# seqan/slimm

Hardware: AMD Instinct MI355X
Metric: M alignment-records/sec -> final profile (higher is better)
Workload: dtype u32

## Files before the change

slimm_amd/csrc/kernels.h:

```cpp
#pragma once
#include <hip/hip_runtime.h>
#include <stdint.h>

#include <string>
#include <vector>

#include "record_filter.h"
#include "tile_plan.h"

#if defined(__HIP_DEVICE_COMPILE__)
#define SLIMM_PIN_VGPR(x) asm volatile("" : "+v"(x))
#else
#define SLIMM_PIN_VGPR(x) (void)(x)
#endif

namespace slimm {

enum {
    CNT_V = 0,
    CNT_M = 1,
    CNT_P = 2,
    CNT_ERR = 3,
    CNT_PAIRS = 4,
    CNT_REDO = 5,
    CNT_ITEMS = 10,
    CNT_ITEMS2 = 6,
    CNT_ANYGB = 8,
    CNT_MODE = 7,
    CNT_SPLIT = 9,
    CNT_FALLBACK = 11,
    CNT_PEAK = 13,
    CNT_WORDS = 32
};
enum { ERR_REF_RANGE = 1, ERR_RUN_LENGTH = 2, ERR_PAIR_OVERFLOW = 4, ERR_KEY_COLLISION = 8 };

#if defined(__HIPCC__)
__device__ __forceinline__ uint32_t wave_sum_dpp(uint32_t v) {
    v += __builtin_amdgcn_update_dpp(0u, v, 0x111, 0xf, 0xf, true);
    v += __builtin_amdgcn_update_dpp(0u, v, 0x112, 0xf, 0xf, true);
    v += __builtin_amdgcn_update_dpp(0u, v, 0x114, 0xf, 0xf, true);
    v += __builtin_amdgcn_update_dpp(0u, v, 0x118, 0xf, 0xf, true);
    v += __builtin_amdgcn_update_dpp(0u, v, 0x142, 0xa, 0xf, true);
    v += __builtin_amdgcn_update_dpp(0u, v, 0x143, 0xc, 0xf, true);
    return __builtin_amdgcn_readlane(v, 63);
}
#endif

struct PackArgs {
    const uint32_t* src[4] = {nullptr, nullptr, nullptr, nullptr};
    uint32_t n[4] = {0, 0, 0, 0};
    uint32_t reps[4] = {1, 1, 1, 1};
    int sum_k = -1;
    const uint32_t* sum_off = nullptr;
    const uint32_t* sum_idx = nullptr;
};
constexpr uint32_t kPackBytes8 = 0xffffffffu;
#ifdef __HIPCC__
__device__ __forceinline__ uint32_t packed_word(const PackArgs& pack, int k, uint32_t i) {
    uint32_t v = 0;
    if (k == pack.sum_k) {
        for (uint32_t j = pack.sum_off[i]; j < pack.sum_off[i + 1]; ++j) v += pack.src[k][pack.sum_idx[j]];
    } else if (pack.reps[k] == kPackBytes8) {
        const uint2 b = reinterpret_cast<const uint2*>(pack.src[k])[i];
#pragma unroll
        for (int l = 0; l < 4; ++l) {
            v |= ((b.x >> (8 * l)) & 0xffu) ? (1u << l) : 0u;
            v |= ((b.y >> (8 * l)) & 0xffu) ? (16u << l) : 0u;
        }
    } else {
        for (uint32_t rep = 0; rep < pack.reps[k]; ++rep) v |= pack.src[k][static_cast<size_t>(rep) * pack.n[k] + i];
    }
    return v;
}
#endif
constexpr uint32_t kMarkBytes = 8;
struct ZeroArgs {
    uint32_t* p[5] = {nullptr, nullptr, nullptr, nullptr, nullptr};
    uint32_t n[5] = {0, 0, 0, 0, 0};
    uint64_t* p64 = nullptr;
    uint32_t n64 = 0;
    uint32_t* cp_dst = nullptr;
    const uint32_t* cp_src = nullptr;
    uint32_t cp_n = 0;
    uint32_t* cp2_dst = nullptr;
    const uint32_t* cp2_src = nullptr;
    uint32_t cp2_n = 0;
};
void launch_zero(hipStream_t st, const ZeroArgs& z);
void launch_copy_out(hipStream_t st, uint32_t* dst_host, const uint32_t* src, uint32_t n);

struct DeviceRecords {
    const uint64_t* key = nullptr;
    const int32_t* ref = nullptr;
    const int32_t* pos = nullptr;
    const uint16_t* flag = nullptr;
    const uint32_t* check = nullptr;
    uint32_t n = 0;
    bool packed = false;
    bool marked = false;
};


constexpr uint32_t kSlotRecs = 768;
constexpr int kFrontBlock = 64;
constexpr uint32_t kMaxRefs = (1u << 26) - 2u;
constexpr uint32_t kMaxBins = 0x7ffffff0u;
constexpr uint32_t kRef16Max = 1u << 15;
struct TargetRefs {
    void* p = nullptr;
    bool ref16 = false;
};
uint32_t front_slots(uint32_t n_records);
void launch_front_raw(hipStream_t st, const DeviceRecords& in, uint32_t n_refs, const uint2* geo, uint32_t half_read,
                      uint32_t bin_width, uint32_t* counters, TargetRefs tgt_ref, uint32_t* tgt_gbin, uint4* slots,
                      hipEvent_t t0 = nullptr, hipEvent_t t1 = nullptr);
void launch_front_sorted(hipStream_t st, uint32_t n_upper, const uint64_t* ident, const uint2* pay,
                         uint32_t* counters, TargetRefs tgt_ref, uint32_t* tgt_gbin, uint4* slots,
                         const uint32_t* cchk = nullptr);

void launch_check_grouping(hipStream_t st, const uint64_t* key, uint32_t n, uint64_t id_mask, uint64_t* tab, uint32_t tab_mask,
                           uint32_t* n_split);
void launch_hist(hipStream_t st, const uint32_t* tgt_gbin, const uint4* slots, uint32_t nslots, uint32_t* counters,
                 uint32_t* tail, uint32_t* cov, uint32_t* ucov, bool count_mapped);
void launch_ref_stats(hipStream_t st, const uint32_t* a, const uint32_t* b, const uint32_t* bin_off, uint32_t n_refs,
                      uint32_t* out, const PackArgs* pack = nullptr);
struct FilterArgs {
    TargetRefs tgt_ref;
    const uint32_t* tgt_gbin = nullptr;
    const uint4* slots = nullptr;
    uint32_t nslots = 0;
    const void* rows16 = nullptr;
    const uint32_t* taxon_flat = nullptr;
    uint32_t taxon_shift = 0;
    const uint32_t* lin_dense = nullptr;
    const uint8_t* valid = nullptr;
    const uint32_t* valid_bits = nullptr;
    uint32_t* redo = nullptr;
    uint32_t* sel = nullptr;
    const uint32_t* slot_rbase = nullptr;
    const uint32_t* slot_bbase = nullptr;
    uint32_t* marks = nullptr;
    uint64_t* pair_tab = nullptr;
    uint64_t* pair_list = nullptr;
    uint32_t pair_mask = 0, taxon_base = 0;
    uint32_t* counters = nullptr;
};
void launch_filter(hipStream_t st, const FilterArgs& a, hipEvent_t t0 = nullptr, hipEvent_t t1 = nullptr);
void launch_sel_atomics(hipStream_t st, const uint32_t* sel, uint32_t n_reads, uint32_t taxon_base, uint32_t* ucov2,
                        uint32_t* lca_count);
void launch_slot_read_prefix(hipStream_t st, const uint4* slots, uint32_t nslots, uint32_t* rbase, uint32_t* bbase);
void launch_partials_pack(hipStream_t st, const uint32_t* block_b, uint32_t R, uint32_t T, uint32_t* out);
void launch_merge_slices(hipStream_t st, const uint32_t* recv, uint32_t n_ranks, uint64_t slice_words, uint32_t lo_bin,
                         uint32_t hi_bin, const uint32_t* bin_off, uint32_t n_refs, const uint32_t* own_stats,
                         const uint32_t* own_tail, uint32_t* vec);
void launch_nonzero_bits(hipStream_t st, const uint32_t* bins, uint64_t n_bins, uint32_t* bits);
void launch_merge_summary(hipStream_t st, const uint32_t* gathered, uint64_t rank_stride, uint32_t n_ranks,
                          const uint32_t* bin_off, uint32_t n_refs, uint64_t bits_off_cov, uint64_t bits_off_ucov,
                          uint32_t* out_stats, const uint32_t* counters);

struct SlotValues {
    const uint32_t* vals = nullptr;
    const uint4* slots = nullptr;
    uint32_t nslots = 0;
    bool per_read = false;
};
struct Totals {
    const uint4* part = nullptr;
    uint32_t nparts = 0;
    uint32_t* tail = nullptr;
};
constexpr uint32_t kCountFold = 2;
constexpr uint32_t kSuperTiles = 64;
constexpr uint32_t kMaxSuper = 8192;
constexpr uint32_t kPartSub = 32768;
struct BitsLayout {
    uint64_t* base = nullptr;
    uint32_t tps = 1;
    uint64_t slice_w64 = 0;
};
struct TileTables {
    uint32_t tile_shift;
    uint16_t* bucket;
    uint32_t *tile_count, *tile_base, *tile_cursor, *split_tiles;
    uint32_t reps, stride;
    uint4 *tile_items, *part_items;
    uint32_t *mid, *sup_cursor, *matrix;
    uint4* tot_part;
    const uint32_t* tile_ref0;
    uint32_t* counters;
    uint32_t entries;
};
struct TileSample {
    uint32_t stride = 1, k = 0;
    uint32_t flag = 0;
    bool gated = false;
};
namespace tiles13 {
#include "tile_api.inc"
}
namespace tiles14 {
#include "tile_api.inc"
}
#define TILES(shift, call) ((shift) == ::slimm::kTileShiftLarge ? ::slimm::tiles14::call : ::slimm::tiles13::call)

constexpr uint32_t kBamPiece = 16384;
constexpr uint32_t kBamSlots = kBamPiece / 36 + 2;
constexpr uint32_t kBamPieceBad = 1;
constexpr uint64_t kBamSlack = 16ull << 20;
struct BamPiece {
    uint32_t guess, stop, count, flags;
    uint32_t base, pad[3];
};
struct BamWindowResult {
    uint32_t n_records, stop, bad, last_piece;
};
struct BamCarry {
    uint32_t have, len;
    uint32_t short_starts, short_to_plain, last_short, pad;
    uint8_t name[256];
};
uint32_t bam_pieces(uint64_t n_bytes);
void launch_bam_find(hipStream_t st, const uint8_t* bytes, uint64_t lo, uint64_t end, uint32_t n_refs, BamPiece* pieces, uint32_t* offs,
                     BamWindowResult* result);
struct DecodeFilter {
    slimm_record_filter f;
    uint32_t* counts;
};
void launch_bam_decode(hipStream_t st, const uint8_t* bytes, uint64_t lo, uint64_t end, const BamPiece* pieces, const uint32_t* offs,
                       BamCarry* carry, const BamWindowResult* result, bool marked, uint64_t out_at, uint64_t* key, int32_t* ref,
                       int32_t* pos, uint16_t* flag, uint32_t* check, slimm_record_filter filter, uint32_t* filter_counts);
void launch_bam_first_guess(hipStream_t st, const uint8_t* bytes, uint64_t lo, uint64_t hi, uint64_t end, uint32_t n_refs,
                            unsigned long long* out);
void launch_bam_name_at(hipStream_t st, const uint8_t* bytes, uint64_t o, BamCarry* name);
void launch_split_join(hipStream_t st, const BamCarry* left, const BamCarry* first, BamCarry* right, uint32_t* word0);
void launch_split_first_start(hipStream_t st, const uint32_t* words, uint64_t n, unsigned long long* out);

void launch_bam_scan(hipStream_t st, BamPiece* pieces, uint32_t n_pieces, uint64_t end, BamWindowResult* result, uint32_t sam_lo);

constexpr uint32_t kSamPiece = 8192;
constexpr uint32_t kSamPieceSkip = 2;
static_assert(kSamPiece / 22 + 2 <= kBamSlots, "a SAM piece's lines fit the offsets of a BAM piece");
struct SamRefEntry {
    uint64_t hash;
    int32_t ref;
    uint32_t name_off, name_len, pad;
};
uint32_t sam_pieces(uint64_t n_bytes);
uint64_t sam_name_hash(const char* s, size_t n);
void launch_sam_find(hipStream_t st, const uint8_t* bytes, uint64_t lo, uint64_t end, BamPiece* pieces, uint32_t* offs, BamWindowResult* result);
void launch_sam_end_line(hipStream_t st, uint8_t* bytes, uint64_t lo, uint64_t end, uint32_t* ended);
void launch_sam_decode(hipStream_t st, const uint8_t* bytes, uint64_t lo, uint64_t end, const BamPiece* pieces, const uint32_t* offs,
                       BamCarry* carry, const BamWindowResult* result, bool marked, uint64_t out_at, uint64_t* key, int32_t* ref, int32_t* pos,
                       uint16_t* flag, uint32_t* check, const SamRefEntry* table, uint32_t table_mask, const uint8_t* names,
                       slimm_record_filter filter, uint32_t* filter_counts);
void launch_sam_first_newline(hipStream_t st, const uint8_t* bytes, uint64_t lo, uint64_t hi, unsigned long long* out);
void launch_sam_name_at(hipStream_t st, const uint8_t* bytes, uint64_t o, uint64_t end, BamCarry* name);

struct BgzfBlock {
    uint64_t src, dst;
    uint32_t csize, isize;
    uint32_t crc;
    uint32_t tok;
};
__host__ __device__ inline uint32_t bgzf_token_room(uint32_t isize) { return isize / 3u + isize / 256u + 8u; }
constexpr uint32_t kBgzfTail = 1024;
constexpr uint32_t kBgzfMaxGrid = 512;
struct InflateInfo {
    uint32_t n_tok;
    uint32_t flag;
};
uint32_t bgzf_inflate_grid(uint32_t n_blocks);
size_t bgzf_lanes_scratch_bytes(uint32_t grid);
size_t bgzf_inflate_scratch_bytes(uint32_t n_blocks, uint64_t token_words);
void launch_bgzf_inflate(hipStream_t st, const uint8_t* comp, const BgzfBlock* blocks, uint32_t n_blocks, uint8_t* out, void* scratch,
                         uint32_t* status);
void launch_bgzf_inflate_lanes(hipStream_t st, const uint8_t* comp, const BgzfBlock* blocks, uint32_t n_blocks, uint8_t* out, void* scratch,
                               uint32_t grid, uint32_t* status, const InflateInfo* info);
bool bgzf_parse_blocks(const uint8_t* bytes, uint64_t n_bytes, uint64_t dst0, std::vector<BgzfBlock>& out, uint64_t& inflated,
                       std::string& err);

constexpr uint32_t kGroupMaxBits = 11;
constexpr uint32_t kGroupDefaultBits = 8;
constexpr uint32_t kGroupMaxGrid = 512;
constexpr uint32_t kGroupMaxPasses = 6;
struct GroupPlan {
    uint32_t passes = 1, bits = 8;
    uint32_t widths[kGroupMaxPasses] = {8, 0, 0, 0, 0, 0};
    uint32_t width = 8;
    uint32_t grid = kGroupMaxGrid;
};
GroupPlan group_plan(uint32_t n_records);
size_t group_hist_words(const GroupPlan& g);
struct GroupArrays {
    uint64_t* ident = nullptr;
    uint2* pay = nullptr;
    uint32_t* chk = nullptr;
};
struct GroupJob {
    GroupPlan plan;
    DeviceRecords in;
    uint32_t n_refs = 0;
    const uint2* geo = nullptr;
    uint32_t half_read = 0, bin_width = 0;
    uint32_t* counters = nullptr;
    GroupArrays a, t;
    uint32_t* hist = nullptr;
};
void launch_group_count(hipStream_t st, const GroupJob& j, uint32_t pass);
void launch_group_scan(hipStream_t st, const GroupJob& j, uint32_t pass);
void launch_group_scatter(hipStream_t st, const GroupJob& j, uint32_t pass);
void launch_group_finish(hipStream_t st, const GroupJob& j);
int group_init();

}
```

slimm_amd/csrc/tile_api.inc:

```
int tile_hist_setup(uint32_t ntiles);
uint32_t tile_count_grid(uint32_t grid);
uint32_t part_items_upper(uint32_t ntiles, uint32_t n_upper);
uint32_t tile_items_upper(uint32_t ntiles, uint32_t n_upper);
void launch_tile_count(hipStream_t st, uint32_t grid, uint32_t ntiles, const SlotValues& in, const TileTables& t, bool totals,
                       bool matrix, const TileSample& sm = TileSample());
void launch_matrix_prefix(hipStream_t st, uint32_t grid, uint32_t ntiles, const TileTables& t);
void launch_tile_scan(hipStream_t st, uint32_t ntiles, const TileTables& t, uint32_t reps, bool two_level, const Totals& tot,
                      uint32_t tile_sub, const TileSample& sm = TileSample());
void launch_tile_scatter(hipStream_t st, TilePath path, uint32_t grid, uint32_t ntiles, uint32_t n_upper, const SlotValues& in,
                         const TileTables& t, uint32_t* cov, uint32_t* ucov, const Totals& tot, uint32_t tile_sub,
                         const TileSample& sm = TileSample());
void launch_tile_fit(hipStream_t st, uint32_t ntiles, const TileTables& t, uint32_t* cov, uint32_t* ucov, uint32_t tile_sub,
                     const TileSample& sm);
void launch_tile_hist(hipStream_t st, uint32_t ntiles, uint32_t n_upper, const TileTables& t, uint32_t* cov, uint32_t* ucov,
                      const uint32_t* bin_off, uint32_t n_refs, uint32_t* stats, const BitsLayout& bits, uint32_t store_from,
                      bool wide, bool stretched = false);
void launch_pack(hipStream_t st, uint32_t* dst, const PackArgs& pack, const TileTables* t = nullptr, const uint32_t* a = nullptr,
                 const uint32_t* b = nullptr, const uint32_t* bin_off = nullptr, uint32_t n_refs = 0, uint32_t* stats = nullptr,
                 const BitsLayout& bits = BitsLayout());
```

slimm_amd/csrc/tile_bucketing.hip:

```cpp
#include "context.h"

namespace slimm {

const char* TileBucketing::init(const uint32_t* bin_off, uint32_t n_refs) {
    if (plan.matrix_allowed &&
        tile_matrix.ensure(static_cast<size_t>(TILES(layout.tile_shift, tile_count_grid(kGrid))) * plan.stride) != hipSuccess)
        return "the tile count matrix";
    const size_t rep_words = static_cast<size_t>(plan.reps) * plan.stride;
    if (tile_count.ensure(rep_words) != hipSuccess || tile_base.ensure(layout.ntiles2 + 1) != hipSuccess ||
        tile_cursor.ensure(rep_words) != hipSuccess || split_tiles.ensure(layout.ntiles2 + 1) != hipSuccess)
        return "tile tables";
    std::vector<uint32_t> ref0(layout.ntiles2 + 1, n_refs);
    uint32_t r = 0;
    for (uint32_t t = 0; t < layout.ntiles2; ++t) {
        const uint64_t t0 = static_cast<uint64_t>(t) * layout.tile_bins();
        if (t0 >= bin_off[n_refs]) break;
        while (r + 1 < n_refs && bin_off[r + 1] <= t0) ++r;
        ref0[t] = r;
    }
    if (d_tile_ref0.ensure(ref0.size()) != hipSuccess ||
        hipMemcpy(d_tile_ref0.p, ref0.data(), ref0.size() * 4, hipMemcpyHostToDevice) != hipSuccess)
        return "tile tables";
    return nullptr;
}

hipError_t TileBucketing::reserve(uint32_t n) {
    hipError_t e = tot_part.ensure(kGrid);
    if (e != hipSuccess || !plan.use_tiles) return e;
    entries = static_cast<uint32_t>(std::min<uint64_t>(tile_bucket_entries(layout, plan, n), 0xffffffffull));
    if ((e = bucket.ensure(entries)) != hipSuccess || (e = mid.ensure(n + 1)) != hipSuccess) return e;
    if ((e = tile_items.ensure(TILES(layout.tile_shift, tile_items_upper(layout.ntiles2, n)) + 1)) != hipSuccess) return e;
    if ((e = part_items.ensure(TILES(layout.tile_shift, part_items_upper(layout.ntiles2, n)) + 1)) != hipSuccess) return e;
    return sup_cursor.ensure(kMaxSuper);
}

static_assert(K_TILE_SCAN2 - K_TILE_COUNT2 == K_TILE_SCAN - K_TILE_COUNT && K_TILE_SCATTER2 - K_TILE_COUNT2 == K_TILE_SCATTER - K_TILE_COUNT,
              "phase B's timer ids follow phase A's in the same order");

void bucket(slimm_ctx* c, const TileJob& job) {
    const TileRun& r = job.run;
    const TileTables t = c->tiles.tables(c->counters.p);
    const uint32_t grid = TileBucketing::kGrid;
    const int B = r.phase == TilePhase::B ? 1 : 0;
    const int id = B ? K_TILE_COUNT2 : K_TILE_COUNT;
    hipStream_t st = c->stream;
    const bool matrix = r.path == TilePath::Matrix;
    TileSample sm;
    sm.stride = r.sample;
    sm.k = r.sample_k;
    sm.flag = CNT_FALLBACK + B;
    c->tiles.sampled[B] = r.sample;
    {
        KernelTimer tm(c, id);
        TILES(t.tile_shift, launch_tile_count(st, grid, r.ntiles, job.values, t, job.tail != nullptr, matrix, sm));
        if (matrix) TILES(t.tile_shift, launch_matrix_prefix(st, grid, r.ntiles, t));
    }
    Totals tot;
    if (job.tail) tot = Totals{t.tot_part, TILES(t.tile_shift, tile_count_grid(grid)), job.tail};
    if (r.path != TilePath::Fused) {
        KernelTimer tm(c, id + (K_TILE_SCAN - K_TILE_COUNT));
        TILES(t.tile_shift, launch_tile_scan(st, r.ntiles, t, r.scan_reps, r.scan_two_level, tot, r.tile_sub, sm));
    }
    KernelTimer tm(c, id + (K_TILE_SCATTER - K_TILE_COUNT));
    TILES(t.tile_shift, launch_tile_scatter(st, r.path, grid, r.ntiles, job.n_upper, job.values, t, job.a, job.b, tot, r.tile_sub, sm));
    if (r.sample <= 1) return;
    TILES(t.tile_shift, launch_tile_fit(st, r.ntiles, t, job.a, job.b, r.tile_sub, sm));
    sm.stride = 1;
    sm.gated = true;
    TILES(t.tile_shift, launch_tile_count(st, grid, r.ntiles, job.values, t, false, false, sm));
    TILES(t.tile_shift, launch_tile_scan(st, r.ntiles, t, r.scan_reps, r.scan_two_level, Totals(), r.tile_sub, sm));
    TILES(t.tile_shift, launch_tile_scatter(st, r.path, grid, r.ntiles, job.n_upper, job.values, t, job.a, job.b, Totals(), r.tile_sub, sm));
}

void histogram(slimm_ctx* c, const TileJob& job) {
    const TileRun& r = job.run;
    KernelTimer tm(c, r.phase == TilePhase::B ? K_TILE_HIST2 : K_TILE_HIST);
    const TileTables t = c->tiles.tables(c->counters.p);
    TILES(t.tile_shift, launch_tile_hist(c->stream, r.ntiles, job.n_upper, t, job.a, job.b, c->d_bin_off.p, c->R, job.stats, job.bits,
                                         job.store_from, r.wide_hist, r.sample > 1));
}

}
```

slimm_amd/csrc/tile_hist.hip:

```cpp
#include <hip/hip_runtime.h>
#include <type_traits>
#include <stdint.h>

#include <algorithm>

#include "kernels.h"

#ifndef SLIMM_TILE_SHIFT
#error "tile_hist.hip is compiled with -DSLIMM_TILE_SHIFT=13 or 14"
#endif
#if SLIMM_TILE_SHIFT == 13
#define SLIMM_TILE_NS tiles13
#elif SLIMM_TILE_SHIFT == 14
#define SLIMM_TILE_NS tiles14
#else
#error "a bucket entry holds 14 bits of bin and the unique bit"
#endif

namespace slimm {
namespace SLIMM_TILE_NS {

constexpr uint32_t kTileShift = SLIMM_TILE_SHIFT;
constexpr uint32_t kTileBins = 1u << kTileShift;
constexpr uint32_t kSuperShift = kTileShift + 6;
constexpr uint32_t kSuperMask = (1u << kSuperShift) - 1;

#if defined(EXP) && EXP == 8
__device__ unsigned long long g_prof_t[8 * 4096];
#define TPROF_T(x) const unsigned long long x = __builtin_readcyclecounter()
#define TPROF_ADD(slot, a, b) if ((threadIdx.x & 63) == 0) g_prof_t[(blockIdx.x * 8 + (threadIdx.x >> 6)) * 8 + slot] += (b) - (a)
#else
#define TPROF_T(x)
#define TPROF_ADD(slot, a, b)
#endif
#if defined(EXP) && EXP == 9
__device__ unsigned long long g_prof_t[8 * 4096];
#define HPROF_T(x) const unsigned long long x = __builtin_readcyclecounter()
#define HPROF_ADD(slot, a, b) if (threadIdx.x == 0) g_prof_t[(blockIdx.x & 4095u) * 8 + slot] += (b) - (a)
#else
#define HPROF_T(x)
#define HPROF_ADD(slot, a, b)
#endif

constexpr int kTBlock = 512;
constexpr uint32_t kTileMask = kTileBins - 1;
constexpr uint32_t kScanStaged = kScanStagedTiles;

struct SlotWalk {
    const uint4* slots;
    uint32_t d_end, d_wave;
    bool d_first;
    uint32_t s, s_end;
    uint32_t step;
    uint32_t base, left;
    uint32_t sum_f, sum_h, sum_v;
    bool per_read;
    uint4 nd;
};

constexpr uint32_t kPiece = 256;
constexpr uint32_t kPieceMax = 256;
__device__ __forceinline__ SlotWalk slot_walk(const uint4* slots, uint32_t nslots, bool per_read, uint32_t fold = 1,
                                              uint32_t wg = blockIdx.x) {
    SlotWalk w;
    w.slots = slots;
    w.step = blockDim.x >> 6;
    w.d_end = 0;
    w.d_wave = __builtin_amdgcn_readfirstlane(threadIdx.x >> 6);
    w.d_first = true;
    w.nd = make_uint4(0u, 0u, 0u, 0u);
    if (!slots) {
        const uint32_t units = gridDim.x * fold;
        const uint32_t per_unit = ((nslots + units - 1u) / units + kPieceMax - 1u) & ~(kPieceMax - 1u);
        const uint64_t lo64 = static_cast<uint64_t>(wg) * per_unit * fold;
        const uint32_t lo = static_cast<uint32_t>(min<uint64_t>(lo64, nslots));
        w.base = lo;
        w.d_end = static_cast<uint32_t>(min<uint64_t>(lo64 + static_cast<uint64_t>(per_unit) * fold, nslots));
        w.left = 0;
        w.s = w.s_end = 0;
        w.sum_f = w.sum_h = w.sum_v = 0;
        w.per_read = per_read;
        return w;
    }
    const uint32_t per_wg = (nslots + gridDim.x * fold - 1) / (gridDim.x * fold) * fold;
    const uint32_t lo = min(wg * per_wg, nslots);
    w.s = lo + __builtin_amdgcn_readfirstlane(threadIdx.x >> 6);
    w.s_end = min(lo + per_wg, nslots);
    w.nd = w.s < w.s_end ? slots[w.s] : make_uint4(0u, 0u, 0u, 0u);
    w.base = 0;
    w.left = 0;
    w.sum_f = w.sum_h = w.sum_v = 0;
    w.per_read = per_read;
    return w;
}

__device__ __forceinline__ uint32_t xcd_logical_id() {
    static_assert(kTileReps == 8 && kCountFold == 2, "the permutation below is written for 8 copies, 2 halves");
    const uint32_t b = blockIdx.x;
    if (gridDim.x % 16u) return b;
    const uint32_t q = b >> 3, x = b & 7u;
    return 16u * (q >> 1) + 2u * x + (q & 1u);
}

__device__ __forceinline__ uint32_t slot_next(SlotWalk& w, uint32_t* base, uint32_t cap = kPiece) {
    if (!w.slots) {
        if (w.d_first) {
            w.base += w.d_wave * cap;
            w.d_first = false;
        }
        if (w.base >= w.d_end) return 0u;
        const uint32_t n = min(cap, w.d_end - w.base);
        *base = w.base;
        w.base += w.step * cap;
        return n;
    }
    while (w.left == 0u) {
        if (w.s >= w.s_end) return 0u;
        const uint4 d = w.nd;
        w.s += w.step;
        if (w.s < w.s_end) w.nd = w.slots[w.s];
        w.base = d.x;
        w.left = w.per_read ? d.z : d.y;
        w.sum_f += d.y;
        w.sum_h += d.z;
        w.sum_v += d.w;
    }
    const uint32_t n = min(w.left, cap);
    *base = w.base;
    w.base += n;
    w.left -= n;
    return n;
}

struct __attribute__((packed, aligned(4))) Quad {
    uint32_t a, b, c, d;
};
__device__ __forceinline__ void piece_load(const uint32_t* __restrict__ vals, uint32_t base, uint32_t n, uint32_t lane,
                                           uint32_t* v) {
    const uint32_t i = 4u * lane;
    Quad q{0xffffffffu, 0xffffffffu, 0xffffffffu, 0xffffffffu};
    if (i < n) q = *reinterpret_cast<const Quad*>(vals + base + i);
    v[0] = i < n ? q.a : 0xffffffffu;
    v[1] = i + 1u < n ? q.b : 0xffffffffu;
    v[2] = i + 2u < n ? q.c : 0xffffffffu;
    v[3] = i + 3u < n ? q.d : 0xffffffffu;
}

__device__ __forceinline__ bool piece_load_packed(SlotWalk& w, const uint32_t* __restrict__ vals, uint32_t lane, uint32_t* v) {
    uint32_t base_a = 0, base_b = 0;
    const uint32_t n_a = slot_next(w, &base_a);
    const uint32_t q_a = (n_a + 3u) >> 2;
    const uint32_t n_b = (n_a != 0u && q_a < 64u) ? slot_next(w, &base_b, 4u * (64u - q_a)) : 0u;
    const bool second = lane >= q_a;
    const uint32_t i = 4u * (second ? lane - q_a : lane), n = second ? n_b : n_a;
    Quad q{0xffffffffu, 0xffffffffu, 0xffffffffu, 0xffffffffu};
    if (i < n) q = *reinterpret_cast<const Quad*>(vals + (second ? base_b : base_a) + i);
    v[0] = i < n ? q.a : 0xffffffffu;
    v[1] = i + 1u < n ? q.b : 0xffffffffu;
    v[2] = i + 2u < n ? q.c : 0xffffffffu;
    v[3] = i + 3u < n ? q.d : 0xffffffffu;
    return n_a != 0u;
}

__device__ __forceinline__ uint32_t tile_of(uint32_t v) { return (v & 0x7fffffffu) >> kTileShift; }

template <int kMode>
__global__ __launch_bounds__(kTBlock * kCountFold) void k_tile_count(const uint32_t* __restrict__ vals, const uint4* __restrict__ slots,
                                                        uint32_t nslots, int per_read, uint32_t ntiles,
                                                        uint32_t* __restrict__ tile_count_all, uint32_t reps,
                                                        uint32_t rep_stride, uint4* __restrict__ part,
                                                        uint32_t* __restrict__ matrix, uint32_t S,
                                                        const uint32_t* __restrict__ gate) {
    HIP_DYNAMIC_SHARED(uint32_t, s_hist)
    __shared__ uint32_t s_sum[3];
    if (kMode == 2 && *gate == 0u) return;
    if (threadIdx.x < 3) s_sum[threadIdx.x] = 0;
    uint32_t* __restrict__ tile_count = tile_count_all + static_cast<size_t>(blockIdx.x % reps) * rep_stride;
    for (uint32_t i = threadIdx.x; i < ntiles; i += kTBlock * kCountFold) s_hist[i] = 0;
    __syncthreads();
    const uint32_t lane = threadIdx.x & 63u;
    SlotWalk w = slot_walk(slots, nslots, per_read != 0, kCountFold);
    if (kMode == 1) {
        const uint32_t waves = blockDim.x >> 6, wave = w.d_wave;
        const uint32_t first = tile_sample_first(wave, waves, S);
        if (slots) {
            const uint32_t lo = w.s - wave;
            if (part) {
                uint32_t v = 0, h = 0, f = 0;
                for (uint32_t s = lo + threadIdx.x; s < w.s_end; s += blockDim.x) {
                    const uint4 d = slots[s];
                    f += d.y;
                    h += d.z;
                    v += d.w;
                }
                v = wave_sum_dpp(v);
                h = wave_sum_dpp(h);
                f = wave_sum_dpp(f);
                if (lane == 0u) {
                    atomicAdd(&s_sum[0], v);
                    atomicAdd(&s_sum[1], h);
                    atomicAdd(&s_sum[2], f);
                }
            }
            w.s = lo + first;
            w.nd = w.s < w.s_end ? slots[w.s] : make_uint4(0u, 0u, 0u, 0u);
        } else {
            w.d_wave = first;
        }
        w.step = tile_sample_step(waves, S);
    }
    while (true) {
        uint32_t v[16];
        bool any = false;
#pragma unroll
        for (int u = 0; u < 4; ++u) {
            uint32_t base = 0;
            const uint32_t n = slot_next(w, &base);
            any = any || n != 0u;
            piece_load(vals, base, n, lane, v + 4 * u);
        }
        if (!any) break;
#pragma unroll
        for (int u = 0; u < 16; ++u)
            if (v[u] != 0xffffffffu) atomicAdd(&s_hist[tile_of(v[u])], 1u);
    }
    if (kMode != 1 && part && lane == 0u) {
        atomicAdd(&s_sum[0], w.sum_v);
        atomicAdd(&s_sum[1], w.sum_h);
        atomicAdd(&s_sum[2], w.sum_f);
    }
    __syncthreads();
    if (part && threadIdx.x == 0) part[blockIdx.x] = make_uint4(s_sum[0], s_sum[1], s_sum[2], 0u);
    if (matrix) {
        uint32_t* __restrict__ row = matrix + static_cast<size_t>(blockIdx.x) * rep_stride;
        for (uint32_t i = threadIdx.x; i < ntiles; i += kTBlock * kCountFold) row[i] = s_hist[i];
        return;
    }
    for (uint32_t i = threadIdx.x; i < ntiles; i += kTBlock * kCountFold) {
        uint32_t h = s_hist[i];
        if (h) atomicAdd(&tile_count[i], h);
    }
}

__global__ __launch_bounds__(256) void k_matrix_prefix(uint32_t* __restrict__ matrix, uint32_t nrows, uint32_t ntiles,
                                                       uint32_t row_stride, uint32_t* __restrict__ total) {
    const uint32_t t = blockIdx.x * 256u + threadIdx.x;
    if (t >= ntiles) return;
    uint32_t run = 0;
    uint32_t r = 0;
    for (; r + 16u <= nrows; r += 16u) {
        uint32_t v[16];
#pragma unroll
        for (uint32_t u = 0; u < 16u; ++u) v[u] = matrix[static_cast<size_t>(r + u) * row_stride + t];
#pragma unroll
        for (uint32_t u = 0; u < 16u; ++u) {
            matrix[static_cast<size_t>(r + u) * row_stride + t] = run;
            run += v[u];
        }
    }
    for (; r < nrows; ++r) {
        const uint32_t v = matrix[static_cast<size_t>(r) * row_stride + t];
        matrix[static_cast<size_t>(r) * row_stride + t] = run;
        run += v;
    }
    total[t] = run;
}

__device__ __forceinline__ void publish_totals(const uint4* __restrict__ part, uint32_t nparts, uint32_t* __restrict__ counters,
                                               uint32_t* __restrict__ tail, uint32_t* s_tot) {
    if (threadIdx.x < 3) s_tot[threadIdx.x] = 0;
    __syncthreads();
    uint32_t v = 0, h = 0, f = 0;
    for (uint32_t i = threadIdx.x; i < nparts; i += blockDim.x) {
        const uint4 p = part[i];
        v += p.x;
        h += p.y;
        f += p.z;
    }
    v = wave_sum_dpp(v);
    h = wave_sum_dpp(h);
    f = wave_sum_dpp(f);
    if ((threadIdx.x & 63u) == 63u) {
        if (v) atomicAdd(&s_tot[0], v);
        if (h) atomicAdd(&s_tot[1], h);
        if (f) atomicAdd(&s_tot[2], f);
    }
    __syncthreads();
    if (threadIdx.x == 0) {
        counters[CNT_V] = s_tot[0];
        counters[CNT_M] = s_tot[1];
        counters[CNT_P] = s_tot[2];
        if (tail) {
            tail[0] = s_tot[0];
            tail[1] = s_tot[1];
            tail[2] = s_tot[2];
        }
    }
}

template <bool kSampled>
__global__ __launch_bounds__(1024) void k_tile_scan(uint32_t* __restrict__ tile_count, uint32_t ntiles,
                                                    uint32_t* __restrict__ tile_base, uint32_t* __restrict__ tile_cursor,
                                                    uint4* __restrict__ items, uint32_t* __restrict__ counters,
                                                    uint4* __restrict__ items2, uint32_t* __restrict__ sup_cursor,
                                                    uint32_t* __restrict__ split_tiles, uint32_t reps,
                                                    uint32_t rep_stride, int two_level, const uint4* __restrict__ part,
                                                    uint32_t nparts, uint32_t* __restrict__ tail, uint32_t tile_sub,
                                                    uint32_t S, uint32_t cap_k, uint32_t entries, uint32_t flag, int gated) {
    __shared__ uint2 s_part[1024];
    __shared__ uint32_t s_nsplit;
    __shared__ uint32_t s_tot[3];
    __shared__ unsigned long long s_caps;
    if (gated && counters[flag] == 0u) return;
    constexpr bool sampled = kSampled;
    if (sampled && threadIdx.x == 0) s_caps = 0ull;
    if (sampled) __syncthreads();
    if (part) publish_totals(part, nparts, counters, tail, s_tot);
    __shared__ uint32_t s_cnt[kScanStaged];
    __shared__ uint2 s_wave[16];
    if (threadIdx.x == 0) s_nsplit = 0;
    const uint32_t tid = threadIdx.x;
    const bool kept = ntiles <= 4096 && reps == kTileReps;
    uint32_t keep[4][kTileReps];
    uint2 carry = make_uint2(0u, 0u);
    unsigned long long caps64 = 0ull;
    for (uint32_t c0 = 0; c0 < ntiles; c0 += kScanStaged) {
        const uint32_t n = min(kScanStaged, ntiles - c0);
        uint32_t* tc = tile_count + c0;
        uint32_t* tcur = tile_cursor + c0;
        if (kept) {
#pragma unroll
            for (int q = 0; q < 4; ++q) {
                const uint32_t i = tid + q * 1024;
                if (i >= n) break;
                uint32_t c = 0;
#pragma unroll
                for (uint32_t rep = 0; rep < kTileReps; ++rep) keep[q][rep] = tc[static_cast<size_t>(rep) * rep_stride + i];
                if (sampled) {
#pragma unroll
                    for (uint32_t rep = 0; rep < kTileReps; ++rep) {
                        keep[q][rep] = tile_cap(keep[q][rep], S, cap_k);
                        caps64 += keep[q][rep];
                    }
                }
#pragma unroll
                for (uint32_t rep = 0; rep < kTileReps; ++rep) c += keep[q][rep];
                s_cnt[i] = c;
            }
        } else {
            for (uint32_t i = tid; i < n; i += 1024) {
                uint32_t c = 0;
                if (reps == kTileReps) {
                    uint32_t v[kTileReps];
#pragma unroll
                    for (uint32_t rep = 0; rep < kTileReps; ++rep) v[rep] = tc[static_cast<size_t>(rep) * rep_stride + i];
                    if (sampled) {
#pragma unroll
                        for (uint32_t rep = 0; rep < kTileReps; ++rep) {
                            v[rep] = tile_cap(v[rep], S, cap_k);
                            tc[static_cast<size_t>(rep) * rep_stride + i] = v[rep];
                            caps64 += v[rep];
                        }
                    }
#pragma unroll
                    for (uint32_t rep = 0; rep < kTileReps; ++rep) c += v[rep];
                } else {
                    for (uint32_t rep = 0; rep < reps; ++rep) c += tc[static_cast<size_t>(rep) * rep_stride + i];
                }
                s_cnt[i] = c;
            }
        }
        if (sampled && caps64) atomicAdd(&s_caps, caps64), caps64 = 0ull;
        __syncthreads();
        const uint32_t per = (n + 1023) / 1024;
        const uint32_t lo = min(tid * per, n), hi = min(lo + per, n);
        uint2 sum = make_uint2(0u, 0u);
        for (uint32_t i = lo; i < hi; ++i) {
            const uint32_t c = s_cnt[i];
            sum.x += c;
            sum.y += c ? (c + tile_sub - 1) / tile_sub : 1u;
        }
        {
            const uint32_t lane = tid & 63u, wave = tid >> 6;
            uint2 inc = sum;
#pragma unroll
            for (int o = 1; o < 64; o <<= 1) {
                const uint32_t ax = __shfl_up(inc.x, o, 64), ay = __shfl_up(inc.y, o, 64);
                if (lane >= static_cast<uint32_t>(o)) {
                    inc.x += ax;
                    inc.y += ay;
                }
            }
            if (lane == 63) s_wave[wave] = inc;
            __syncthreads();
            uint2 before = carry;
#pragma unroll
            for (uint32_t w = 0; w < 16; ++w) {
                const uint2 t = s_wave[w];
                if (w < wave) {
                    before.x += t.x;
                    before.y += t.y;
                }
            }
            s_part[tid] = make_uint2(before.x + inc.x, before.y + inc.y);
        }
        uint2 run = make_uint2(s_part[tid].x - sum.x, s_part[tid].y - sum.y);
        for (uint32_t i = lo; i < hi; ++i) {
            const uint32_t c = s_cnt[i];
            const uint32_t pieces = c ? (c + tile_sub - 1) / tile_sub : 1u;
            s_cnt[i] = run.x;
            if (pieces > 1 && !sampled) split_tiles[atomicAdd(&s_nsplit, 1u)] = c0 + i;
            for (uint32_t k = 0; k < pieces && !sampled; ++k) {
                uint32_t a = run.x + k * tile_sub;
                uint32_t b = min(a + tile_sub, run.x + c);
                items[run.y + k] = gated ? make_uint4(c0 + i, a - run.x, b - run.x, pieces) : make_uint4(c0 + i, a, b, pieces);
            }
            run.x += c;
            run.y += pieces;
        }
        __syncthreads();
        if (kept) {
#pragma unroll
            for (int q = 0; q < 4; ++q) {
                const uint32_t i = tid + q * 1024;
                if (i >= n) break;
                uint32_t at = s_cnt[i];
                tile_base[c0 + i] = at;
#pragma unroll
                for (uint32_t rep = 0; rep < kTileReps; ++rep) {
                    const size_t k = static_cast<size_t>(rep) * rep_stride + i;
                    tc[k] = at;
                    tcur[k] = 0;
                    at += keep[q][rep];
                }
            }
        } else {
            for (uint32_t i = tid; i < n; i += 1024) {
                uint32_t at = s_cnt[i];
                tile_base[c0 + i] = at;
                if (reps == kTileReps) {
                    uint32_t v[kTileReps];
#pragma unroll
                    for (uint32_t rep = 0; rep < kTileReps; ++rep) v[rep] = tc[static_cast<size_t>(rep) * rep_stride + i];
#pragma unroll
                    for (uint32_t rep = 0; rep < kTileReps; ++rep) {
                        const size_t k = static_cast<size_t>(rep) * rep_stride + i;
                        tc[k] = at;
                        tcur[k] = 0;
                        at += v[rep];
                    }
                } else {
                    for (uint32_t rep = 0; rep < reps; ++rep) {
                        const size_t k = static_cast<size_t>(rep) * rep_stride + i;
                        const uint32_t cr = tc[k];
                        tc[k] = at;
                        tcur[k] = 0;
                        at += cr;
                    }
                }
            }
        }
        carry = s_part[1023];
        __syncthreads();
    }
    if (tid == 1023) {
        tile_base[ntiles] = carry.x;
        counters[CNT_ITEMS] = sampled ? 0u : carry.y;
        if (sampled) counters[flag] = s_caps > entries ? 1u : 0u;
    }
    __shared__ uint32_t s_n2;
    if (tid == 0) s_n2 = 0;
    __threadfence_block();
    __syncthreads();
    const uint32_t nsup = two_level ? (ntiles + kSuperTiles - 1) / kSuperTiles : 0u;
    for (uint32_t sp = tid; sp < nsup; sp += 1024) {
        sup_cursor[sp] = 0;
        const uint32_t a = tile_base[sp * kSuperTiles];
        const uint32_t b = tile_base[min((sp + 1) * kSuperTiles, ntiles)];
        const uint32_t pieces = (b - a + kPartSub - 1) / kPartSub;
        if (pieces) {
            uint32_t slot = atomicAdd(&s_n2, pieces);
            for (uint32_t q = a; q < b; q += kPartSub) items2[slot++] = make_uint4(sp, q, min(q + kPartSub, b), 0u);
        }
    }
    __syncthreads();
    if (tid == 0) {
        counters[CNT_ITEMS2] = s_n2;
        counters[CNT_SPLIT] = s_nsplit;
    }
}

constexpr int kRoundPieces = 16;
constexpr int kDirectPieces = 32;
constexpr uint32_t kTileSlots = 4096;
constexpr uint32_t kRoundCap = (kTBlock / 64) * kRoundPieces * 64;

template <int kPieces, bool kWide>
__device__ __forceinline__ bool round_load(SlotWalk& w, const uint32_t* __restrict__ vals, uint32_t lane,
                                           uint32_t (&v)[kPieces]) {
    static_assert(kPieces % 4 == 0, "values come four to a lane");
    bool any = false;
    if (kWide) {
#pragma unroll
        for (int k = 0; k < kPieces; k += 4) any = piece_load_packed(w, vals, lane, v + k) || any;
    } else {
#pragma unroll
        for (int k = 0; k < kPieces; ++k) {
            uint32_t base = 0;
            const uint32_t n = slot_next(w, &base, 64u);
            any = any || n != 0u;
            v[k] = lane < n ? vals[base + lane] : 0xffffffffu;
        }
    }
    return any;
}

constexpr uint32_t kEntryBits = kTileShift + 1;
static_assert(kEntryBits <= 16, "bucket entries are 16-bit");
__device__ __forceinline__ uint32_t entry_of(uint32_t v) { return (v & kTileMask) | ((v >> 31) << kTileShift); }

__device__ __forceinline__ uint32_t block_excl_scan_4096(uint32_t* s, uint32_t* s_wtot);

__device__ __forceinline__ void scatter_round_ordered(const uint32_t (&v)[kRoundPieces], uint32_t ntiles,
                                                      const uint32_t* s_mine, uint32_t* __restrict__ tile_cursor,
                                                      uint16_t* __restrict__ bucket, uint32_t* s_cnt, uint32_t* s_loff,
                                                      uint32_t* s_stage, uint32_t* s_wtot) {
    const uint32_t tid = threadIdx.x;
    TPROF_T(p0);
    for (uint32_t i = tid; i < kTileSlots; i += kTBlock) s_cnt[i] = 0;
    __syncthreads();
    TPROF_T(p1);
    TPROF_ADD(1, p0, p1);
    uint32_t r[kRoundPieces];
#pragma unroll
    for (int k = 0; k < kRoundPieces; ++k) r[k] = v[k] != 0xffffffffu ? atomicAdd(&s_cnt[tile_of(v[k])], 1u) : 0u;
    __syncthreads();
    TPROF_T(p2);
    TPROF_ADD(2, p1, p2);
    uint32_t got[kTileSlots / kTBlock];
#pragma unroll
    for (uint32_t j = 0; j < kTileSlots / kTBlock; ++j) {
        const uint32_t i = j * kTBlock + tid;
        const uint32_t h = s_cnt[i];
        s_loff[i] = h;
        got[j] = 0u;
        if (h && i < ntiles) got[j] = atomicAdd(&tile_cursor[i], h);
    }
    __syncthreads();
    TPROF_T(p3);
    TPROF_ADD(3, p2, p3);
    const uint32_t total = block_excl_scan_4096(s_loff, s_wtot);
#pragma unroll
    for (uint32_t j = 0; j < kTileSlots / kTBlock; ++j) {
        const uint32_t i = j * kTBlock + tid;
        s_cnt[i] = got[j] + s_mine[i] - s_loff[i];
    }
    TPROF_T(p4);
    TPROF_ADD(4, p3, p4);
#pragma unroll
    for (int k = 0; k < kRoundPieces; ++k) {
        if (v[k] == 0xffffffffu) continue;
        const uint32_t t = tile_of(v[k]);
        s_stage[s_loff[t] + r[k]] = (t << kEntryBits) | entry_of(v[k]);
    }
    __syncthreads();
    TPROF_T(p5);
    TPROF_ADD(5, p4, p5);
    for (uint32_t j = tid; j < total; j += kTBlock) {
        const uint32_t e = s_stage[j];
        bucket[s_cnt[e >> kEntryBits] + j] = static_cast<uint16_t>(e & ((1u << kEntryBits) - 1u));
    }
    __syncthreads();
    TPROF_T(p6);
    TPROF_ADD(6, p5, p6);
}

template <int kPieces>
__device__ __forceinline__ void scatter_round_direct(const uint32_t (&v)[kPieces], uint32_t ntiles,
                                                     const uint32_t* __restrict__ tile_base,
                                                     uint32_t* __restrict__ tile_cursor, uint16_t* __restrict__ bucket,
                                                     uint32_t* s_hist, uint32_t last) {
    constexpr int kMaxTilesPerThread = 8;
    for (uint32_t i = threadIdx.x; i < ntiles; i += kTBlock) s_hist[i] = 0;
    __syncthreads();
#pragma unroll
    for (int k = 0; k < kPieces; ++k)
        if (v[k] != 0xffffffffu) atomicAdd(&s_hist[tile_of(v[k])], 1u);
    __syncthreads();
    for (uint32_t i0 = 0; i0 < ntiles; i0 += kMaxTilesPerThread * kTBlock) {
        uint32_t got[kMaxTilesPerThread];
#pragma unroll
        for (int j = 0; j < kMaxTilesPerThread; ++j) {
            const uint32_t i = i0 + j * kTBlock + threadIdx.x;
            const uint32_t h = i < ntiles ? s_hist[i] : 0u;
            got[j] = 0u;
            if (h) got[j] = atomicAdd(&tile_cursor[i], h);
        }
#pragma unroll
        for (int j = 0; j < kMaxTilesPerThread; ++j) {
            const uint32_t i = i0 + j * kTBlock + threadIdx.x;
            if (i < ntiles) s_hist[i] = got[j] + tile_base[i];
        }
    }
    __syncthreads();
#pragma unroll
    for (int k = 0; k < kPieces; ++k) {
        if (v[k] == 0xffffffffu) continue;
        const uint32_t pos = atomicAdd(&s_hist[tile_of(v[k])], 1u);
        bucket[min(pos, last)] = static_cast<uint16_t>(entry_of(v[k]));
    }
    __syncthreads();
}

template <int kPieces = kRoundPieces, bool kWide = true, typename Body>
__device__ __forceinline__ void bucketing_rounds(SlotWalk& walk, const uint32_t* __restrict__ vals, uint32_t* s_more,
                                                 Body body) {
    while (true) {
        uint32_t v[kPieces];
        const bool mine = round_load<kPieces, kWide>(walk, vals, threadIdx.x & 63u, v);
        if ((threadIdx.x & 63u) == 0) s_more[threadIdx.x >> 6] = mine ? 1u : 0u;
        __syncthreads();
        uint32_t any = 0;
#pragma unroll
        for (int w = 0; w < kTBlock / 64; ++w) any |= s_more[w];
        __syncthreads();
        if (!any) break;
        body(v);
    }
}

__device__ __forceinline__ void zero_split_tiles(const uint32_t* tile_base, uint32_t ntiles, uint32_t* __restrict__ cov,
                                                 uint32_t* __restrict__ ucov, uint32_t tile_sub) {
    for (uint32_t tile = blockIdx.x; tile < ntiles; tile += gridDim.x) {
        if (tile_base[tile + 1] - tile_base[tile] <= tile_sub) continue;
        uint4* oc = reinterpret_cast<uint4*>(cov + static_cast<size_t>(tile) * kTileBins);
        uint4* ou = reinterpret_cast<uint4*>((ucov ? ucov : cov) + static_cast<size_t>(tile) * kTileBins);
        const uint4 z = make_uint4(0, 0, 0, 0);
        for (uint32_t i = threadIdx.x; i < kTileBins / 4; i += kTBlock) {
            oc[i] = z;
            if (ucov) ou[i] = z;
        }
    }
}

__global__ __launch_bounds__(kTBlock) void k_tile_scatter(const uint32_t* __restrict__ vals, const uint4* __restrict__ slots,
                                                          uint32_t nslots, int per_read, uint32_t ntiles,
                                                          const uint32_t* __restrict__ tile_base,
                                                          uint32_t* __restrict__ tile_cursor_all,
                                                          uint16_t* __restrict__ bucket, uint32_t* __restrict__ cov,
                                                          uint32_t* __restrict__ ucov,
                                                          const uint32_t* __restrict__ rep_base_all, uint32_t reps,
                                                          uint32_t rep_stride, uint32_t tile_sub, uint32_t last,
                                                          const uint32_t* __restrict__ gate) {
    HIP_DYNAMIC_SHARED(uint32_t, s_hist)
    __shared__ uint32_t s_more[kTBlock / 64];
    if (gate && *gate == 0u) return;
    const uint32_t lid = xcd_logical_id();
    const size_t rep_off = static_cast<size_t>((lid / kCountFold) % reps) * rep_stride;
    uint32_t* __restrict__ tile_cursor = tile_cursor_all + rep_off;
    const uint32_t* __restrict__ rep_base = rep_base_all + rep_off;
    zero_split_tiles(tile_base, ntiles, cov, ucov, tile_sub);
    SlotWalk walk = slot_walk(slots, nslots, per_read != 0, 1, lid);
    bucketing_rounds<kDirectPieces, false>(walk, vals, s_more, [&](const uint32_t (&v)[kDirectPieces]) {
        scatter_round_direct(v, ntiles, rep_base, tile_cursor, bucket, s_hist, last);
    });
}

#ifndef SLIMM_BIG_PIECES
#define SLIMM_BIG_PIECES 24
#endif
constexpr int kBigBlock = kTBlock * kCountFold;
constexpr int kBigPieces = SLIMM_BIG_PIECES;
constexpr uint32_t kBigRound = kBigBlock * kBigPieces;
static_assert(kBigPieces % 8 == 0, "values come four to a lane; the rounds' LDS operations in batches of eight");
template <int kE>
__global__ __launch_bounds__(kBigBlock) void k_tile_scatter_big(const uint32_t* __restrict__ vals, const uint4* __restrict__ slots,
                                                                uint32_t nslots, int per_read, uint32_t ntiles,
                                                                const uint32_t* __restrict__ tile_base,
                                                                uint32_t* __restrict__ tile_cursor_all,
                                                                uint16_t* __restrict__ bucket, uint32_t* __restrict__ cov,
                                                                uint32_t* __restrict__ ucov,
                                                                const uint32_t* __restrict__ rep_base_all, uint32_t reps,
                                                                uint32_t rep_stride, uint32_t tile_sub, uint32_t last,
                                                                const uint32_t* __restrict__ gate) {
    HIP_DYNAMIC_SHARED(uint32_t, s_dyn)
    __shared__ uint32_t s_more[kBigBlock / 64], s_wtot[kBigBlock / 64];
    constexpr uint32_t kNoTile = kE * kBigBlock;
    if (gate && *gate == 0u) return;
    static_assert(kBigPieces * (kBigBlock / 64) < 65536 && kBigRound < 65536, "ranks are packed as 16-bit halves");
    uint32_t* const s_tab = s_dyn;
    uint32_t* const s_dst = s_dyn + kNoTile + 64;
    uint32_t* const s_stage = s_dst + kNoTile + 64;
    const uint32_t tid = threadIdx.x, lane = tid & 63u, wave = tid >> 6;
    const uint32_t no_tile = kNoTile + lane;
    const size_t rep_off = static_cast<size_t>(blockIdx.x % reps) * rep_stride;
    uint32_t* __restrict__ tile_cursor = tile_cursor_all + rep_off;
    const uint32_t* __restrict__ rep_base = rep_base_all + rep_off;
    uint32_t at[kE];
#pragma unroll
    for (int u = 0; u < kE; ++u) {
        const uint32_t i = u * kBigBlock + tid;
        at[u] = rep_base[i < ntiles ? i : 0u];
    }
    TPROF_T(q0);
    if (tid < kTBlock) zero_split_tiles(tile_base, ntiles, cov, ucov, tile_sub);
    SlotWalk walk = slot_walk(slots, nslots, per_read != 0, kCountFold);
    uint32_t v[kBigPieces];
    bool mine = round_load<kBigPieces, true>(walk, vals, lane, v);
    if (lane == 0u) s_more[wave] = mine ? 1u : 0u;
#pragma unroll
    for (int u = 0; u < kE; ++u) s_tab[u * kBigBlock + tid] = 0u;
    if (tid < 64u) s_tab[kNoTile + tid] = 0u, s_dst[kNoTile + tid] = 0u;
    __syncthreads();
    TPROF_T(q1);
    if (wave < 8u) TPROF_ADD(0, q0, q1);
    while (true) {
        TPROF_T(p1);
        uint32_t any = 0;
#pragma unroll
        for (int w = 0; w < kBigBlock / 64; ++w) any |= s_more[w];
        if (!any) break;
        uint32_t r2[kBigPieces / 2];
#pragma unroll
        for (int k0 = 0; k0 < kBigPieces; k0 += 8) {
            uint32_t r[8];
#pragma unroll
            for (int k = 0; k < 8; ++k) r[k] = atomicAdd(&s_tab[v[k0 + k] != 0xffffffffu ? tile_of(v[k0 + k]) : no_tile], 1u);
#pragma unroll
            for (int k = 0; k < 8; k += 2) r2[(k0 + k) / 2] = r[k] | (r[k + 1] << 16);
            __builtin_amdgcn_sched_barrier(0);
        }
        __syncthreads();
        TPROF_T(p2);
        if (wave < 8u) TPROF_ADD(2, p1, p2);
        uint32_t got[kE], sum = 0;
        {
            uint32_t h[kE];
            uint32_t* __restrict__ cursor = tile_cursor + (any >> 1);
#pragma unroll
            for (int u = 0; u < kE; ++u) {
                const uint32_t i = u * kBigBlock + tid;
                h[u] = s_tab[i];
                got[u] = 0u;
                if (h[u] && i < ntiles) got[u] = atomicAdd(&cursor[i], h[u]);
                sum += h[u];
            }
            uint32_t inc = sum;
#pragma unroll
            for (int o = 1; o < 64; o <<= 1) {
                const uint32_t a = __shfl_up(inc, o, 64);
                if (lane >= static_cast<uint32_t>(o)) inc += a;
            }
            if (lane == 63u) s_wtot[wave] = inc;
            sum = inc - sum;
            __syncthreads();
            uint32_t run = sum;
#pragma unroll
            for (int w = 0; w < kBigBlock / 64; ++w)
                if (w < static_cast<int>(wave)) run += s_wtot[w];
#pragma unroll
            for (int u = 0; u < kE; ++u) {
                s_tab[u * kBigBlock + tid] = run;
                s_dst[u * kBigBlock + tid] = at[u] - run;
                run += h[u];
            }
        }
        uint32_t total = 0;
#pragma unroll
        for (int w = 0; w < kBigBlock / 64; ++w) total += s_wtot[w];
        if (tid < 64u) s_tab[kNoTile + tid] = 0u;
        __syncthreads();
        TPROF_T(p3);
        if (wave < 8u) TPROF_ADD(3, p2, p3);
#pragma unroll
        for (int k0 = 0; k0 < kBigPieces; k0 += 8) {
            uint32_t at_[8];
#pragma unroll
            for (int k = 0; k < 8; ++k) at_[k] = s_tab[v[k0 + k] != 0xffffffffu ? tile_of(v[k0 + k]) : no_tile];
#pragma unroll
            for (int k = 0; k < 8; ++k) {
                const uint32_t t = tile_of(v[k0 + k]);
                const uint32_t rk = (k & 1) ? r2[(k0 + k) / 2] >> 16 : r2[(k0 + k) / 2] & 0xffffu;
                s_stage[v[k0 + k] != 0xffffffffu ? at_[k] + rk : kBigRound + lane] = (t << kEntryBits) | entry_of(v[k0 + k]);
            }
        }
        TPROF_T(p4);
        if (wave < 8u) TPROF_ADD(4, p3, p4);
#pragma unroll
        for (int u = 0; u < kE; ++u) s_dst[u * kBigBlock + tid] += got[u];
        TPROF_T(p4b);
        if (wave < 8u) TPROF_ADD(1, p4, p4b);
        mine = round_load<kBigPieces, true>(walk, vals, lane, v);
        if (lane == 0u) s_more[wave] = mine ? 1u : 0u;
        __syncthreads();
        TPROF_T(p5);
        if (wave < 8u) TPROF_ADD(5, p4b, p5);
#pragma unroll
        for (int u = 0; u < kE; ++u) s_tab[u * kBigBlock + tid] = 0u;
#pragma unroll
        for (int k0 = 0; k0 < kBigPieces; k0 += 4) {
            if (static_cast<uint32_t>(k0) * kBigBlock >= total) break;
            uint32_t e[4], d[4];
#pragma unroll
            for (int k = 0; k < 4; ++k) e[k] = s_stage[(k0 + k) * kBigBlock + tid];
#pragma unroll
            for (int k = 0; k < 4; ++k) d[k] = s_dst[min(e[k] >> kEntryBits, kNoTile)];
#pragma unroll
            for (int k = 0; k < 4; ++k) {
                const uint32_t j = (k0 + k) * kBigBlock + tid;
                if (j < total) bucket[min(d[k] + j, last)] = static_cast<uint16_t>(e[k] & ((1u << kEntryBits) - 1u));
            }
        }
        __syncthreads();
        TPROF_T(p6);
        if (wave < 8u) TPROF_ADD(6, p5, p6);
    }
    TPROF_T(q2);
    if (wave < 8u) TPROF_ADD(7, q0, q2);
}
constexpr size_t big_lds_bytes(int e) { return (2u * static_cast<size_t>(e) * kBigBlock + kBigRound + 192u) * 4u; }
constexpr int kBigE = 6;
static_assert(big_lds_bytes(kBigE) <= 160u * 1024u - 256u, "the two tables and the stage share a CU's LDS");
static_assert(kBigE * kBigBlock == kBigRoundTiles, "kernels.h tells the context which layouts take these rounds");
static_assert(kTileShift + 1 + 14 <= 32, "a stage entry holds the tile and the bucket entry");

__global__ __launch_bounds__(kTBlock * kCountFold) void k_tile_scatter_matrix(
    const uint32_t* __restrict__ vals, const uint4* __restrict__ slots, uint32_t nslots, int per_read, uint32_t ntiles,
    const uint32_t* __restrict__ tile_base, const uint32_t* __restrict__ matrix, uint32_t row_stride,
    uint16_t* __restrict__ bucket, uint32_t* __restrict__ cov, uint32_t* __restrict__ ucov, uint32_t tile_sub) {
    HIP_DYNAMIC_SHARED(uint32_t, s_cur)
    const uint32_t* __restrict__ row = matrix + static_cast<size_t>(blockIdx.x) * row_stride;
    for (uint32_t i = threadIdx.x; i < ntiles; i += kTBlock * kCountFold) s_cur[i] = tile_base[i] + row[i];
    if (threadIdx.x < kTBlock) zero_split_tiles(tile_base, ntiles, cov, ucov, tile_sub);
    __syncthreads();
    const uint32_t lane = threadIdx.x & 63u;
    SlotWalk w = slot_walk(slots, nslots, per_read != 0, kCountFold);
    while (true) {
        uint32_t v[8];
        bool any = false;
#pragma unroll
        for (int u = 0; u < 8; u += 4) {
            uint32_t base = 0;
            const uint32_t n = slot_next(w, &base);
            any = any || n != 0u;
            piece_load(vals, base, n, lane, v + u);
        }
        if (!any) break;
#pragma unroll
        for (int u = 0; u < 8; ++u) {
            if (v[u] == 0xffffffffu) continue;
            const uint32_t pos = atomicAdd(&s_cur[tile_of(v[u])], 1u);
            bucket[pos] = static_cast<uint16_t>(entry_of(v[u]));
        }
    }
}

constexpr uint32_t kFusedTiles = 4096;
__device__ __forceinline__ uint32_t block_excl_scan_4096(uint32_t* s, uint32_t* s_wtot) {
    const uint32_t tid = threadIdx.x, lane = tid & 63u, wave = tid >> 6;
    uint32_t v[8], sum = 0;
#pragma unroll
    for (int u = 0; u < 8; ++u) {
        v[u] = s[tid * 8 + u];
        sum += v[u];
    }
    uint32_t inc = sum;
#pragma unroll
    for (int o = 1; o < 64; o <<= 1) {
        const uint32_t a = __shfl_up(inc, o, 64);
        if (lane >= static_cast<uint32_t>(o)) inc += a;
    }
    if (lane == 63) s_wtot[wave] = inc;
    __syncthreads();
    uint32_t before = 0, total = 0;
#pragma unroll
    for (int w = 0; w < 8; ++w) {
        const uint32_t t = s_wtot[w];
        if (w < static_cast<int>(wave)) before += t;
        total += t;
    }
    uint32_t run = before + inc - sum;
#pragma unroll
    for (int u = 0; u < 8; ++u) {
        s[tid * 8 + u] = run;
        run += v[u];
    }
    __syncthreads();
    return total;
}

__global__ __launch_bounds__(kTBlock) void k_tile_scatter_fused(const uint32_t* __restrict__ vals,
                                                                const uint4* __restrict__ slots, uint32_t nslots,
                                                                int per_read, uint32_t* __restrict__ counters,
                                                                uint32_t ntiles, const uint32_t* __restrict__ tile_count_all,
                                                                uint32_t* __restrict__ tile_cursor_all,
                                                                uint16_t* __restrict__ bucket, uint32_t* __restrict__ cov,
                                                                uint32_t* __restrict__ ucov, uint32_t rep_stride,
                                                                uint4* __restrict__ items, uint32_t* __restrict__ split_tiles,
                                                                const uint4* __restrict__ part, uint32_t nparts,
                                                                uint32_t* __restrict__ tail, uint32_t tile_sub) {
    __shared__ uint32_t s_stage[kRoundCap];
    __shared__ uint32_t s_mine[kFusedTiles];
    __shared__ uint32_t s_cnt[kFusedTiles];
    __shared__ uint32_t s_loff[kFusedTiles];
    static_assert(kRoundCap >= kFusedTiles + 1, "the stage doubles as the tile_base table");
    static_assert(kFusedScanTiles + 32 <= kFusedTiles, "room for the small arrays behind the last tile");
    uint32_t* const s_wtot = s_mine + kFusedTiles - 32;
    uint32_t* const s_more = s_mine + kFusedTiles - 24;
    uint32_t& s_nsplit = s_mine[kFusedTiles - 16];
    uint32_t* const s_base = s_stage;
    const uint32_t tid = threadIdx.x;
    const uint32_t lid = xcd_logical_id();
    const uint32_t my_rep = (lid / kCountFold) % kTileReps;
    TPROF_T(q0);
    if (tid == 0) s_nsplit = 0;
#pragma unroll
    for (int q = 0; q < 8; ++q) {
        const uint32_t i = q * kTBlock + tid;
        uint32_t c = 0, mine = 0;
        if (i < ntiles) {
            uint32_t v[kTileReps];
#pragma unroll
            for (uint32_t rep = 0; rep < kTileReps; ++rep) v[rep] = tile_count_all[static_cast<size_t>(rep) * rep_stride + i];
#pragma unroll
            for (uint32_t rep = 0; rep < kTileReps; ++rep) {
                if (rep < my_rep) mine += v[rep];
                c += v[rep];
            }
        }
        s_base[i] = c;
        if (i < ntiles) s_mine[i] = mine;
    }
    __syncthreads();
    const uint32_t total = block_excl_scan_4096(s_base, s_wtot);
    if (tid == 0) s_base[kFusedTiles] = total;
#pragma unroll
    for (int q = 0; q < 8; ++q) {
        const uint32_t i = q * kTBlock + tid;
        if (i < ntiles) s_mine[i] += s_base[i];
    }
    __syncthreads();
    if (blockIdx.x == 0) {
        if (part) publish_totals(part, nparts, counters, tail, s_loff);
        uint32_t* s_piece = s_cnt;
#pragma unroll
        for (int q = 0; q < 8; ++q) {
            const uint32_t i = q * kTBlock + tid;
            const uint32_t c = i < ntiles ? s_base[i + 1] - s_base[i] : 0u;
            s_piece[i] = i < ntiles ? (c ? (c + tile_sub - 1) / tile_sub : 1u) : 0u;
        }
        __syncthreads();
        const uint32_t n_items = block_excl_scan_4096(s_piece, s_wtot);
        for (uint32_t i = tid; i < ntiles; i += kTBlock) {
            const uint32_t b0 = s_base[i], c = s_base[i + 1] - b0;
            const uint32_t pieces = c ? (c + tile_sub - 1) / tile_sub : 1u;
            if (pieces > 1) split_tiles[atomicAdd(&s_nsplit, 1u)] = i;
            for (uint32_t k = 0; k < pieces; ++k) {
                const uint32_t lo = b0 + k * tile_sub;
                items[s_piece[i] + k] = make_uint4(i, lo, min(lo + tile_sub, b0 + c), pieces);
            }
        }
        __syncthreads();
        if (tid == 0) {
            counters[CNT_ITEMS] = n_items;
            counters[CNT_ITEMS2] = 0;
            counters[CNT_SPLIT] = s_nsplit;
        }
    }
    zero_split_tiles(s_base, ntiles, cov, ucov, tile_sub);
    __syncthreads();
    uint32_t* __restrict__ tile_cursor = tile_cursor_all + static_cast<size_t>(my_rep) * rep_stride;
    SlotWalk walk = slot_walk(slots, nslots, per_read != 0, 1, lid);
    TPROF_T(q1);
    TPROF_ADD(0, q0, q1);
    bucketing_rounds(walk, vals, s_more, [&](const uint32_t (&v)[kRoundPieces]) {
        scatter_round_ordered(v, ntiles, s_mine, tile_cursor, bucket, s_cnt, s_loff, s_stage, s_wtot);
    });
    TPROF_T(q2);
    TPROF_ADD(7, q0, q2);
}

__global__ __launch_bounds__(kTBlock) void k_part_super(const uint32_t* __restrict__ vals, const uint4* __restrict__ slots,
                                                        uint32_t nslots, int per_read, uint32_t ntiles,
                                                        const uint32_t* __restrict__ tile_base,
                                                        uint32_t* __restrict__ sup_cursor, uint32_t* __restrict__ mid,
                                                        uint32_t* __restrict__ cov, uint32_t* __restrict__ ucov,
                                                        uint32_t tile_sub) {
    __shared__ uint32_t s_cur[kMaxSuper];
    __shared__ uint32_t s_more[kTBlock / 64];
    const uint32_t nsup = (ntiles + kSuperTiles - 1) / kSuperTiles;
    zero_split_tiles(tile_base, ntiles, cov, ucov, tile_sub);
    SlotWalk walk = slot_walk(slots, nslots, per_read != 0);
    bucketing_rounds(walk, vals, s_more, [&](const uint32_t (&v)[kRoundPieces]) {
        for (uint32_t i = threadIdx.x; i < nsup; i += kTBlock) s_cur[i] = 0;
        __syncthreads();
#pragma unroll
        for (int k = 0; k < kRoundPieces; ++k)
            if (v[k] != 0xffffffffu) atomicAdd(&s_cur[(v[k] & 0x7fffffffu) >> kSuperShift], 1u);
        __syncthreads();
        for (uint32_t i = threadIdx.x; i < nsup; i += kTBlock) {
            const uint32_t h = s_cur[i];
            if (h) s_cur[i] = tile_base[i * kSuperTiles] + atomicAdd(&sup_cursor[i], h);
        }
        __syncthreads();
#pragma unroll
        for (int k = 0; k < kRoundPieces; ++k) {
            if (v[k] == 0xffffffffu) continue;
            const uint32_t g = v[k] & 0x7fffffffu;
            const uint32_t pos = atomicAdd(&s_cur[g >> kSuperShift], 1u);
            mid[pos] = (g & kSuperMask) | ((v[k] >> 31) << kSuperShift);
        }
        __syncthreads();
    });
}

__global__ __launch_bounds__(kTBlock) void k_part_tile(const uint32_t* __restrict__ mid, const uint4* __restrict__ items2,
                                                       const uint32_t* __restrict__ counters,
                                                       const uint32_t* __restrict__ tile_base,
                                                       uint32_t* __restrict__ tile_cursor, uint32_t ntiles,
                                                       uint16_t* __restrict__ bucket) {
    __shared__ uint32_t s_cur[kSuperTiles];
    if (blockIdx.x >= counters[CNT_ITEMS2]) return;
    const uint4 it = items2[blockIdx.x];
    const uint32_t sup = it.x, lo = it.y, hi = it.z;
    const uint32_t tile0 = sup * kSuperTiles;
    if (threadIdx.x < kSuperTiles) s_cur[threadIdx.x] = 0;
    __syncthreads();
    for (uint32_t e0 = lo; e0 < hi; e0 += 4 * kTBlock) {
        uint32_t v[4];
#pragma unroll
        for (int u = 0; u < 4; ++u) {
            uint32_t e = e0 + u * kTBlock + threadIdx.x;
            v[u] = (e < hi) ? mid[e] : 0xffffffffu;
        }
#pragma unroll
        for (int u = 0; u < 4; ++u)
            if (v[u] != 0xffffffffu) atomicAdd(&s_cur[(v[u] & kSuperMask) >> kTileShift], 1u);
    }
    __syncthreads();
    if (threadIdx.x < kSuperTiles) {
        const uint32_t h = s_cur[threadIdx.x], tile = tile0 + threadIdx.x;
        if (h && tile < ntiles) s_cur[threadIdx.x] = tile_base[tile] + atomicAdd(&tile_cursor[tile], h);
    }
    __syncthreads();
    for (uint32_t e0 = lo; e0 < hi; e0 += 4 * kTBlock) {
        uint32_t v[4];
#pragma unroll
        for (int u = 0; u < 4; ++u) {
            uint32_t e = e0 + u * kTBlock + threadIdx.x;
            v[u] = (e < hi) ? mid[e] : 0xffffffffu;
        }
#pragma unroll
        for (int u = 0; u < 4; ++u) {
            if (v[u] == 0xffffffffu) continue;
            const uint32_t local = v[u] & kSuperMask;
            uint32_t pos = atomicAdd(&s_cur[local >> kTileShift], 1u);
            bucket[pos] = static_cast<uint16_t>((local & kTileMask) | (((v[u] >> kSuperShift) & 1u) ? kTileBins : 0u));
        }
    }
}

__global__ __launch_bounds__(1024) void k_tile_fit(uint32_t* rep_base, const uint32_t* __restrict__ tile_base,
                                                   const uint32_t* __restrict__ cursor,
                                                   uint32_t ntiles, uint32_t rep_stride, uint4* __restrict__ items,
                                                   uint32_t* __restrict__ split_tiles, uint32_t* __restrict__ counters,
                                                   uint32_t* __restrict__ cov, uint32_t* __restrict__ ucov, uint32_t tile_sub,
                                                   uint32_t flag, uint32_t peak) {
    __shared__ uint32_t s_cnt[kScanStaged];
    __shared__ uint2 s_wave[16];
    __shared__ uint32_t s_over, s_peak, s_nsplit;
    const uint32_t tid = threadIdx.x;
    const uint32_t raised = counters[flag];
    if (blockIdx.x == 0) {
        if (tid == 0) s_over = 0u, s_peak = 0u, s_nsplit = 0u;
        __syncthreads();
        uint32_t over = 0u, pk = 0u;
        for (uint32_t i = tid; i < ntiles; i += 1024u) {
            uint32_t b[kTileReps + 1], f[kTileReps], c = 0;
#pragma unroll
            for (uint32_t rep = 0; rep < kTileReps; ++rep) {
                b[rep] = rep_base[static_cast<size_t>(rep) * rep_stride + i];
                f[rep] = cursor[static_cast<size_t>(rep) * rep_stride + i];
            }
            b[kTileReps] = tile_base[i + 1];
#pragma unroll
            for (uint32_t rep = 0; rep < kTileReps; ++rep) {
                const uint32_t cap = b[rep + 1] - b[rep];
                if (f[rep] > cap) over = 1u;
                if (f[rep]) pk = max(pk, static_cast<uint32_t>(min(4.0e9f, 1024.0f * static_cast<float>(f[rep]) / static_cast<float>(max(cap, 1u)))));
                c += f[rep];
            }
            s_cnt[i] = c;
        }
        if (over) atomicOr(&s_over, 1u);
        if (pk) atomicMax(&s_peak, pk);
        __syncthreads();
        if (tid == 0) counters[peak] = s_peak;
        if (raised | s_over) {
            if (tid == 0) counters[flag] = 1u;
            for (uint32_t i = tid; i < kTileReps * rep_stride; i += 1024u) rep_base[i] = 0u;
            return;
        }
        const uint32_t per = (ntiles + 1023u) / 1024u;
        const uint32_t lo = min(tid * per, ntiles), hi = min(lo + per, ntiles);
        uint32_t mine = 0;
        for (uint32_t i = lo; i < hi; ++i) {
            const uint32_t c = s_cnt[i];
            mine += c ? (c + tile_sub - 1u) / tile_sub : 1u;
        }
        const uint32_t lane = tid & 63u, wave = tid >> 6;
        uint32_t inc = mine;
#pragma unroll
        for (int o = 1; o < 64; o <<= 1) {
            const uint32_t a = __shfl_up(inc, o, 64);
            if (lane >= static_cast<uint32_t>(o)) inc += a;
        }
        if (lane == 63u) s_wave[wave] = make_uint2(inc, 0u);
        __syncthreads();
        uint32_t at = inc - mine, total = 0;
#pragma unroll
        for (uint32_t w = 0; w < 16u; ++w) {
            const uint32_t t = s_wave[w].x;
            if (w < wave) at += t;
            total += t;
        }
        for (uint32_t i = lo; i < hi; ++i) {
            const uint32_t c = s_cnt[i];
            const uint32_t pieces = c ? (c + tile_sub - 1u) / tile_sub : 1u;
            if (pieces > 1u) split_tiles[atomicAdd(&s_nsplit, 1u)] = i;
            for (uint32_t k = 0; k < pieces; ++k) items[at + k] = make_uint4(i, k * tile_sub, min((k + 1u) * tile_sub, c), pieces);
            at += pieces;
        }
        __syncthreads();
        if (tid == 0) {
            counters[CNT_ITEMS] = total;
            counters[CNT_SPLIT] = s_nsplit;
        }
    }
    __shared__ uint32_t s_zero[64], s_nzero;
    const uint32_t share = (ntiles + gridDim.x - 1u) / gridDim.x;
    for (uint32_t t0 = blockIdx.x * share; t0 < min(ntiles, (blockIdx.x + 1u) * share); t0 += 64u) {
        __syncthreads();
        if (tid == 0) s_nzero = 0u;
        __syncthreads();
        const uint32_t mine = t0 + tid;
        if (tid < 64u && mine < min(ntiles, (blockIdx.x + 1u) * share)) {
            uint32_t c = 0;
#pragma unroll
            for (uint32_t rep = 0; rep < kTileReps; ++rep) c += cursor[static_cast<size_t>(rep) * rep_stride + mine];
            if (c > tile_sub) s_zero[atomicAdd(&s_nzero, 1u)] = mine;
        }
        __syncthreads();
        for (uint32_t z = 0; z < s_nzero; ++z) {
            const uint32_t tile = s_zero[z];
            uint4* oc = reinterpret_cast<uint4*>(cov + static_cast<size_t>(tile) * kTileBins);
            uint4* ou = reinterpret_cast<uint4*>((ucov ? ucov : cov) + static_cast<size_t>(tile) * kTileBins);
            const uint4 z4 = make_uint4(0, 0, 0, 0);
            for (uint32_t i = tid; i < kTileBins / 4; i += 1024u) {
                oc[i] = z4;
                if (ucov) ou[i] = z4;
            }
        }
    }
}

constexpr uint32_t kPackWords = kTileBins / 2;
static_assert(kTileSub < 65536, "packed 16-bit counts in k_tile_hist");
template <bool kPacked>
__device__ __forceinline__ uint4 tile_load4(const uint32_t* s, uint32_t bin) {
    if (!kPacked) return *reinterpret_cast<const uint4*>(s + bin);
    const uint4 w = *reinterpret_cast<const uint4*>(s + (bin & (kPackWords - 1)));
    return bin & kPackWords ? make_uint4(w.x >> 16, w.y >> 16, w.z >> 16, w.w >> 16)
                            : make_uint4(w.x & 0xffffu, w.y & 0xffffu, w.z & 0xffffu, w.w & 0xffffu);
}
template <bool kPacked>
__device__ __forceinline__ uint32_t tile_load1(const uint32_t* s, uint32_t bin) {
    if (!kPacked) return s[bin];
    const uint32_t w = s[bin & (kPackWords - 1)];
    return bin & kPackWords ? w >> 16 : w & 0xffffu;
}
template <bool kPacked>
__device__ __forceinline__ void tile_count(uint32_t* s, uint32_t bin) {
    if (kPacked)
        atomicAdd(&s[bin & (kPackWords - 1)], bin & kPackWords ? 0x10000u : 1u);
    else
        atomicAdd(&s[bin], 1u);
}

template <bool kPacked, uint32_t kWaves>
__device__ __forceinline__ void tile_nonzero_bits(const uint32_t* s_a, uint32_t tile, const BitsLayout& bl, uint32_t array) {
    const uint32_t lane = threadIdx.x & 63u, wave = threadIdx.x >> 6;
    uint64_t* dst = bl.base + (static_cast<uint64_t>(tile / bl.tps) * 2 + array) * bl.slice_w64 +
                    static_cast<uint64_t>(tile % bl.tps) * (kTileBins / 64);
    constexpr uint32_t kPart = kTileBins / kWaves;
#pragma unroll
    for (uint32_t j = 0; j < kPart / 64; ++j) {
        const uint32_t i = wave * kPart + j * 64;
        const uint64_t m = __ballot(tile_load1<kPacked>(s_a, i + lane) != 0u);
        if (lane == 0) dst[i >> 6] = m;
    }
}

constexpr uint32_t kStatRefs = 128;

template <bool kTwo, bool kPacked, uint32_t kWaves>
__device__ __forceinline__ void tile_ref_stats(const uint32_t* s_a, const uint32_t* s_b, uint32_t tile,
                                               const uint32_t* s_off, uint32_t r0,
                                               const uint32_t* __restrict__ bin_off, uint32_t n_refs,
                                               uint32_t* __restrict__ stats, bool want_sum, bool want_nz) {
    const uint32_t lane = threadIdx.x & 63u, wave = threadIdx.x >> 6;
    const uint32_t tile0 = tile * kTileBins;
    const uint32_t t0 = tile0 + wave * (kTileBins / kWaves), t1 = t0 + kTileBins / kWaves;
    static_assert(kTileBins / kWaves <= 32768, "the two non-zero counts of a wave's part share one reduction");
    if (r0 >= n_refs) return;
    uint32_t k = 0;
    {
        const uint32_t staged = min(kStatRefs, n_refs - r0);
        uint32_t lo = 0, hi = staged;
        while (lo + 1 < hi) {
            const uint32_t mid = (lo + hi) >> 1;
            if (s_off[mid] <= t0)
                lo = mid;
            else
                hi = mid;
        }
        k = lo;
        if (k + 1 == staged && staged == kStatRefs)
            while (r0 + k + 1 < n_refs && bin_off[r0 + k + 1] <= t0) ++k;
    }
    auto one_ref = [&](uint32_t r, uint32_t s, uint32_t e) {
        const uint32_t a0 = max(s, t0) - tile0, a1 = min(e, t1) - tile0;
        uint32_t sa = 0, za = 0, sb = 0, zb = 0;
        for (uint32_t i = a0 + lane * 4; i < a1; i += 256) {
            const uint4 v = tile_load4<kPacked>(s_a, i);
            sa += v.x + v.y + v.z + v.w;
            za += (v.x != 0) + (v.y != 0) + (v.z != 0) + (v.w != 0);
            if (kTwo) {
                const uint4 w = tile_load4<kPacked>(s_b, i);
                sb += w.x + w.y + w.z + w.w;
                zb += (w.x != 0) + (w.y != 0) + (w.z != 0) + (w.w != 0);
            }
        }
        sa = wave_sum_dpp(sa);
        za = wave_sum_dpp(kTwo ? za | (zb << 16) : za);
        if (kTwo) {
            sb = wave_sum_dpp(sb);
            zb = za >> 16;
            za &= 0xffffu;
        }
        if (lane == 0) {
            uint32_t* o4 = stats + static_cast<size_t>(r) * 4;
            if (want_sum && sa) atomicAdd(o4 + 0, sa);
            if (want_nz && za) atomicAdd(o4 + 1, za);
            if (kTwo && want_sum && sb) atomicAdd(o4 + 2, sb);
            if (kTwo && want_nz && zb) atomicAdd(o4 + 3, zb);
        }
    };
    const uint32_t staged = min(kStatRefs, n_refs - r0);
    for (; k < staged; ++k) {
        const uint32_t s = s_off[k];
        if (s >= t1) return;
        const uint32_t e = s_off[k + 1];
        if (e > t0) one_ref(r0 + k, s, e);
    }
    for (; r0 + k < n_refs; ++k) {
        const uint32_t s = bin_off[r0 + k];
        if (s >= t1) break;
        const uint32_t e = bin_off[r0 + k + 1];
        if (e > t0) one_ref(r0 + k, s, e);
    }
}

template <bool kTwo, bool kPacked>
constexpr uint32_t hist_lds_bytes() { return (kPacked ? kTileBins / 2 : kTileBins) * 4u * (kTwo ? 2u : 1u); }
template <bool kTwo, bool kPacked>
constexpr uint32_t hist_block() { return hist_lds_bytes<kTwo, kPacked>() > 64u * 1024u ? 1024u : 512u; }
template <bool kTwo, bool kPacked>
constexpr uint32_t hist_waves_per_simd() {
    constexpr uint32_t wgs = std::min<uint32_t>(4u, (160u * 1024u) / (hist_lds_bytes<kTwo, kPacked>() + 1024u));
    return wgs * (hist_block<kTwo, kPacked>() / 64u) / 4u;
}
template <bool kTwo, bool kPacked>
__global__ __launch_bounds__((hist_block<kTwo, kPacked>()), (hist_waves_per_simd<kTwo, kPacked>())) void k_tile_hist(const uint16_t* __restrict__ bucket, const uint4* __restrict__ items,
                                                   const uint32_t* __restrict__ counters, uint32_t* __restrict__ cov,
                                                   uint32_t* __restrict__ ucov, const uint32_t* __restrict__ bin_off,
                                                   uint32_t n_refs, const uint32_t* __restrict__ tile_ref0,
                                                   uint32_t* __restrict__ stats, const BitsLayout bits, uint32_t store_from,
                                                   const uint32_t* __restrict__ rep_base, const uint32_t* __restrict__ rep_fill,
                                                   uint32_t rep_stride) {
    constexpr uint32_t kWords = kPacked ? kPackWords : kTileBins;
    constexpr uint32_t kHB = hist_block<kTwo, kPacked>();
    constexpr uint32_t kWaves = kHB / 64;
    __shared__ uint32_t s_cov[kWords];
    __shared__ uint32_t s_ucov[kTwo ? kWords : 4];
    __shared__ uint32_t s_off[kStatRefs + 1];
    HPROF_T(h0);
    if (blockIdx.x >= counters[CNT_ITEMS]) return;
    const uint4 it = items[blockIdx.x];
    const uint32_t tile = it.x, lo = it.y, hi = it.z;
    const bool whole = it.w == 1;
    if (whole && lo == hi) {
        if (tile >= store_from) {
            uint4* oc = reinterpret_cast<uint4*>(cov + static_cast<size_t>(tile) * kTileBins);
            uint4* ou = reinterpret_cast<uint4*>(ucov + static_cast<size_t>(tile) * kTileBins);
            const uint4 z = make_uint4(0, 0, 0, 0);
            for (uint32_t i = threadIdx.x; i < kTileBins / 4; i += kHB) {
                oc[i] = z;
                if (kTwo) ou[i] = z;
            }
        }
        if (bits.base && threadIdx.x < kTileBins / 64) {
            for (uint32_t array = 0; array < (kTwo ? 2u : 1u); ++array)
                bits.base[(static_cast<uint64_t>(tile / bits.tps) * 2 + array) * bits.slice_w64 +
                          static_cast<uint64_t>(tile % bits.tps) * (kTileBins / 64) + threadIdx.x] = 0ull;
        }
        return;
    }
    uint32_t sb[kTileReps], sf[kTileReps];
#pragma unroll
    for (uint32_t rep = 0; rep < kTileReps; ++rep) {
        sb[rep] = rep_base ? rep_base[static_cast<size_t>(rep) * rep_stride + tile] : 0u;
        sf[rep] = rep_base ? rep_fill[static_cast<size_t>(rep) * rep_stride + tile] : 0u;
    }
    const uint32_t r0 = stats ? tile_ref0[tile] : n_refs;
    const bool stage_off = threadIdx.x <= kStatRefs && r0 < n_refs && r0 + threadIdx.x <= n_refs;
    const uint32_t off_reg = stage_off ? bin_off[r0 + threadIdx.x] : 0u;
    {
        uint4* zc = reinterpret_cast<uint4*>(s_cov);
        uint4* zu = reinterpret_cast<uint4*>(s_ucov);
        const uint4 z = make_uint4(0, 0, 0, 0);
        for (uint32_t i = threadIdx.x; i < kWords / 4; i += kHB) {
            zc[i] = z;
            if (kTwo) zu[i] = z;
        }
    }
    __syncthreads();
    HPROF_T(h2);
    HPROF_ADD(1, h0, h2);
    {
        auto one = [&](uint32_t v) {
            tile_count<kPacked>(s_cov, v & kTileMask);
            if (kTwo && (v & kTileBins)) tile_count<kPacked>(s_ucov, v & kTileMask);
        };
        if (!rep_base) {
            const uint32_t a0 = min(hi, (lo + 7u) & ~7u);
            const uint32_t n8 = (hi - a0) >> 3;
            const uint32_t a1 = a0 + (n8 << 3);
            if (lo + threadIdx.x < a0) one(bucket[lo + threadIdx.x]);
            if (a1 + threadIdx.x < hi) one(bucket[a1 + threadIdx.x]);
            const uint4* __restrict__ b8 = reinterpret_cast<const uint4*>(bucket + a0);
            for (uint32_t i0 = 0; i0 < n8; i0 += 2 * kHB) {
                uint4 q[2];
#pragma unroll
                for (int u = 0; u < 2; ++u) {
                    const uint32_t i = i0 + u * kHB + threadIdx.x;
                    q[u] = i < n8 ? b8[i] : make_uint4(0xffffffffu, 0xffffffffu, 0xffffffffu, 0xffffffffu);
                }
#pragma unroll
                for (int u = 0; u < 2; ++u) {
                    if (i0 + u * kHB + threadIdx.x >= n8) continue;
                    const uint32_t w[4] = {q[u].x, q[u].y, q[u].z, q[u].w};
#pragma unroll
                    for (int k = 0; k < 4; ++k) {
                        one(w[k] & 0xffffu);
                        one(w[k] >> 16);
                    }
                }
            }
        } else {
            const uint32_t(&b)[kTileReps] = sb;
            const uint32_t(&f)[kTileReps] = sf;
            static_assert(kHB >= 16u * kTileReps, "sixteen threads per stretch take its ragged ends");
            uint32_t first[kTileReps], pre[kTileReps + 1];
            uint32_t p = 0, ev = 0xffffffffu;
            pre[0] = 0u;
#pragma unroll
            for (uint32_t rep = 0; rep < kTileReps; ++rep) {
                const uint32_t s = max(lo, p), e = min(hi, p + f[rep]);
                const uint32_t slo = s < e ? b[rep] + (s - p) : 0u, shi = s < e ? b[rep] + (e - p) : 0u;
                const uint32_t a0 = min(shi, (slo + 7u) & ~7u), n8 = (shi - a0) >> 3, a1 = a0 + (n8 << 3);
                first[rep] = a0;
                pre[rep + 1] = pre[rep] + n8;
                if ((threadIdx.x >> 4) == rep) {
                    const uint32_t sub = threadIdx.x & 15u;
                    const uint32_t at = sub < 8u ? slo + sub : a1 + (sub - 8u), end = sub < 8u ? a0 : shi;
                    if (at < end) ev = bucket[at];
                }
                p += f[rep];
            }
            const uint32_t groups = pre[kTileReps];
            for (uint32_t i0 = 0; i0 < groups; i0 += 2 * kHB) {
                uint4 q[2];
#pragma unroll
                for (int u = 0; u < 2; ++u) {
                    const uint32_t g = i0 + u * kHB + threadIdx.x;
                    uint32_t at = first[0], g0 = 0u;
#pragma unroll
                    for (uint32_t rep = 1; rep < kTileReps; ++rep)
                        if (g >= pre[rep]) at = first[rep], g0 = pre[rep];
                    q[u] = g < groups ? *reinterpret_cast<const uint4*>(bucket + at + ((g - g0) << 3))
                                      : make_uint4(0xffffffffu, 0xffffffffu, 0xffffffffu, 0xffffffffu);
                }
                if (i0 == 0u && ev != 0xffffffffu) one(ev);
#pragma unroll
                for (int u = 0; u < 2; ++u) {
                    if (i0 + u * kHB + threadIdx.x >= groups) continue;
                    const uint32_t w[4] = {q[u].x, q[u].y, q[u].z, q[u].w};
#pragma unroll
                    for (int k = 0; k < 4; ++k) {
                        one(w[k] & 0xffffu);
                        one(w[k] >> 16);
                    }
                }
            }
            if (groups == 0u && ev != 0xffffffffu) one(ev);
        }
    }
    HPROF_T(h3);
    HPROF_ADD(2, h2, h3);
    if (stage_off) s_off[threadIdx.x] = off_reg;
    __syncthreads();
    HPROF_T(h4);
    HPROF_ADD(3, h3, h4);
    uint32_t* gc = cov + static_cast<size_t>(tile) * kTileBins;
    uint32_t* gu = ucov + static_cast<size_t>(tile) * kTileBins;
    if (whole) {
        uint4* oc = reinterpret_cast<uint4*>(gc);
        uint4* ou = reinterpret_cast<uint4*>(gu);
        const uint4* sc = reinterpret_cast<const uint4*>(s_cov);
        const uint4* su = reinterpret_cast<const uint4*>(s_ucov);
        if (stats) tile_ref_stats<kTwo, kPacked, kWaves>(s_cov, s_ucov, tile, s_off, r0, bin_off, n_refs, stats, true, true);
        HPROF_T(h5);
        HPROF_ADD(4, h4, h5);
        if (tile >= store_from && !kPacked) {
            for (uint32_t i = threadIdx.x; i < kTileBins / 4; i += kHB) {
                oc[i] = sc[i];
                if (kTwo) ou[i] = su[i];
            }
        } else if (tile >= store_from) {
            for (uint32_t i = threadIdx.x; i < kPackWords / 4; i += kHB) {
                const uint4 w = sc[i];
                oc[i] = make_uint4(w.x & 0xffffu, w.y & 0xffffu, w.z & 0xffffu, w.w & 0xffffu);
                oc[i + kPackWords / 4] = make_uint4(w.x >> 16, w.y >> 16, w.z >> 16, w.w >> 16);
                if (kTwo) {
                    const uint4 x = su[i];
                    ou[i] = make_uint4(x.x & 0xffffu, x.y & 0xffffu, x.z & 0xffffu, x.w & 0xffffu);
                    ou[i + kPackWords / 4] = make_uint4(x.x >> 16, x.y >> 16, x.z >> 16, x.w >> 16);
                }
            }
        }
        if (bits.base) {
            tile_nonzero_bits<kPacked, kWaves>(s_cov, tile, bits, 0);
            if (kTwo) tile_nonzero_bits<kPacked, kWaves>(s_ucov, tile, bits, 1);
        }
        HPROF_T(h6);
        HPROF_ADD(5, h5, h6);
        HPROF_ADD(7, h0, h6);
        return;
    }
    for (uint32_t i = threadIdx.x; !kPacked && i < kTileBins; i += kHB) {
        const uint32_t a = s_cov[i];
        if (a) atomicAdd(&gc[i], a);
        if (kTwo) {
            const uint32_t b2 = s_ucov[i];
            if (b2) atomicAdd(&gu[i], b2);
        }
    }
    for (uint32_t i = threadIdx.x; kPacked && i < kPackWords; i += kHB) {
        const uint32_t a = s_cov[i];
        if (a & 0xffffu) atomicAdd(&gc[i], a & 0xffffu);
        if (a >> 16) atomicAdd(&gc[i + kPackWords], a >> 16);
        if (kTwo) {
            const uint32_t b2 = s_ucov[i];
            if (b2 & 0xffffu) atomicAdd(&gu[i], b2 & 0xffffu);
            if (b2 >> 16) atomicAdd(&gu[i + kPackWords], b2 >> 16);
        }
    }
    if (stats) tile_ref_stats<kTwo, kPacked, kWaves>(s_cov, s_ucov, tile, s_off, r0, bin_off, n_refs, stats, true, false);
}

template <bool kTwo>
__global__ __launch_bounds__(512) void k_pack(uint32_t* __restrict__ dst, const PackArgs pack,
                                              const uint32_t* __restrict__ split_tiles,
                                              const uint32_t* __restrict__ counters, const uint32_t* __restrict__ a,
                                              const uint32_t* __restrict__ b, const uint32_t* __restrict__ bin_off,
                                              uint32_t n_refs, const uint32_t* __restrict__ tile_ref0,
                                              uint32_t* __restrict__ stats, const BitsLayout bits) {
    __shared__ uint32_t s_a[kTileBins];
    __shared__ uint32_t s_b[kTwo ? kTileBins : 4];
    __shared__ uint32_t s_off[kStatRefs + 1];
    {
        const uint32_t gid = blockIdx.x * 512 + threadIdx.x, gsz = gridDim.x * 512;
#pragma unroll
        for (int k = 0; k < 4; ++k) {
            for (uint32_t i = gid; i < pack.n[k]; i += gsz) dst[i] = packed_word(pack, k, i);
            dst += pack.n[k];
        }
    }
    if (!stats) return;
    const uint32_t nsplit = counters[CNT_SPLIT];
    for (uint32_t q = blockIdx.x; q < nsplit; q += gridDim.x) {
        const uint32_t tile = split_tiles[q];
        const uint32_t r0 = tile_ref0[tile];
        __syncthreads();
        if (threadIdx.x <= kStatRefs && r0 < n_refs && r0 + threadIdx.x <= n_refs) s_off[threadIdx.x] = bin_off[r0 + threadIdx.x];
        const uint4* ga = reinterpret_cast<const uint4*>(a + static_cast<size_t>(tile) * kTileBins);
        const uint4* gb = reinterpret_cast<const uint4*>(b + static_cast<size_t>(tile) * kTileBins);
        for (uint32_t i = threadIdx.x; i < kTileBins / 4; i += 512) {
            reinterpret_cast<uint4*>(s_a)[i] = ga[i];
            if (kTwo) reinterpret_cast<uint4*>(s_b)[i] = gb[i];
        }
        __syncthreads();
        tile_ref_stats<kTwo, false, 8>(s_a, s_b, tile, s_off, r0, bin_off, n_refs, stats, false, true);
        if (bits.base) {
            tile_nonzero_bits<false, 8>(s_a, tile, bits, 0);
            if (kTwo) tile_nonzero_bits<false, 8>(s_b, tile, bits, 1);
        }
    }
}

void launch_pack(hipStream_t st, uint32_t* dst, const PackArgs& pack, const TileTables* t, const uint32_t* a, const uint32_t* b,
                 const uint32_t* bin_off, uint32_t n_refs, uint32_t* stats, const BitsLayout& bits) {
    const uint32_t blocks = 256;
    const uint32_t* const split_tiles = t ? t->split_tiles : nullptr;
    const uint32_t* const counters = t ? t->counters : nullptr;
    const uint32_t* const tile_ref0 = t ? t->tile_ref0 : nullptr;
    if (b)
        hipLaunchKernelGGL(k_pack<true>, dim3(blocks), dim3(512), 0, st, dst, pack, split_tiles, counters, a, b, bin_off,
                           n_refs, tile_ref0, stats, bits);
    else
        hipLaunchKernelGGL(k_pack<false>, dim3(blocks), dim3(512), 0, st, dst, pack, split_tiles, counters, a, a, bin_off,
                           n_refs, tile_ref0, stats, bits);
}

uint32_t tile_count_grid(uint32_t grid) { return (grid + kCountFold - 1) / kCountFold; }

int tile_hist_setup(uint32_t ntiles) {
    const size_t bytes = static_cast<size_t>(ntiles) * 4;
    if (!tile_tables_fit_lds(ntiles)) return -1;
    for (auto* k : {k_tile_count<0>, k_tile_count<1>, k_tile_count<2>})
        if (hipFuncSetAttribute(reinterpret_cast<const void*>(k), hipFuncAttributeMaxDynamicSharedMemorySize, static_cast<int>(bytes)) !=
            hipSuccess)
            return -1;
    if ((ntiles + kSuperTiles - 1) / kSuperTiles > kMaxSuper) return -1;
    if (hipFuncSetAttribute(reinterpret_cast<const void*>(k_tile_scatter), hipFuncAttributeMaxDynamicSharedMemorySize,
                            static_cast<int>(bytes)) != hipSuccess)
        return -1;
    if (hipFuncSetAttribute(reinterpret_cast<const void*>(k_tile_scatter_matrix), hipFuncAttributeMaxDynamicSharedMemorySize,
                            static_cast<int>(bytes)) != hipSuccess)
        return -1;
    if (hipFuncSetAttribute(reinterpret_cast<const void*>(k_tile_scatter_big<kBigE>), hipFuncAttributeMaxDynamicSharedMemorySize,
                            static_cast<int>(big_lds_bytes(kBigE))) != hipSuccess)
        return -1;
    return 0;
}

void launch_tile_count(hipStream_t st, uint32_t grid, uint32_t ntiles, const SlotValues& in, const TileTables& t, bool totals,
                       bool matrix, const TileSample& sm) {
    auto* const k = sm.gated ? k_tile_count<2> : sm.stride > 1u ? k_tile_count<1> : k_tile_count<0>;
    hipLaunchKernelGGL(k, dim3(tile_count_grid(grid)), dim3(kTBlock * kCountFold), static_cast<size_t>(ntiles) * 4, st, in.vals, in.slots,
                       in.nslots, in.per_read ? 1 : 0, ntiles, t.tile_count, t.reps, t.stride, totals ? t.tot_part : nullptr,
                       matrix ? t.matrix : nullptr, sm.stride, t.counters + sm.flag);
}

void launch_matrix_prefix(hipStream_t st, uint32_t grid, uint32_t ntiles, const TileTables& t) {
    hipLaunchKernelGGL(k_matrix_prefix, dim3((ntiles + 255u) / 256u), dim3(256), 0, st, t.matrix, tile_count_grid(grid), ntiles,
                       t.stride, t.tile_count);
}

void launch_tile_scan(hipStream_t st, uint32_t ntiles, const TileTables& t, uint32_t reps, bool two_level, const Totals& tot,
                      uint32_t tile_sub, const TileSample& sm) {
    hipLaunchKernelGGL(sm.stride > 1u ? k_tile_scan<true> : k_tile_scan<false>, dim3(1), dim3(1024), 0, st, t.tile_count, ntiles, t.tile_base, t.tile_cursor, t.tile_items,
                       t.counters, t.part_items, t.sup_cursor, t.split_tiles, reps, t.stride, two_level ? 1 : 0, tot.part,
                       tot.nparts, tot.tail, tile_sub, sm.stride, sm.k, t.entries, sm.flag, sm.gated ? 1 : 0);
}

uint32_t part_items_upper(uint32_t ntiles, uint32_t n_upper) {
    return (ntiles + kSuperTiles - 1) / kSuperTiles + n_upper / kPartSub + 1;
}

void launch_tile_scatter(hipStream_t st, TilePath path, uint32_t grid, uint32_t ntiles, uint32_t n_upper, const SlotValues& in,
                         const TileTables& t, uint32_t* cov, uint32_t* ucov, const Totals& tot, uint32_t tile_sub,
                         const TileSample& sm) {
    const bool fit = sm.stride > 1u;
    const uint32_t last = t.entries - 1u;
    const uint32_t* const gate = sm.gated ? t.counters + sm.flag : nullptr;
    if (fit) tile_sub = 0xffffffffu;
    const int per_read = in.per_read ? 1 : 0;
    const size_t lds = static_cast<size_t>(ntiles) * 4;
    switch (path) {
    case TilePath::Fused:
        hipLaunchKernelGGL(k_tile_scatter_fused, dim3(grid), dim3(kTBlock), 0, st, in.vals, in.slots, in.nslots, per_read,
                           t.counters, ntiles, t.tile_count, t.tile_cursor, t.bucket, cov, ucov, t.stride, t.tile_items,
                           t.split_tiles, tot.part, tot.nparts, tot.tail, tile_sub);
        break;
    case TilePath::OrderedRounds:
        hipLaunchKernelGGL(k_tile_scatter_big<kBigE>, dim3(tile_count_grid(grid)), dim3(kBigBlock), big_lds_bytes(kBigE), st,
                           in.vals, in.slots, in.nslots, per_read, ntiles, t.tile_base, t.tile_cursor, t.bucket, cov, ucov,
                           t.tile_count, t.reps, t.stride, tile_sub, last, gate);
        break;
    case TilePath::DirectRounds:
        hipLaunchKernelGGL(k_tile_scatter, dim3(grid), dim3(kTBlock), lds, st, in.vals, in.slots, in.nslots, per_read, ntiles,
                           t.tile_base, t.tile_cursor, t.bucket, cov, ucov, t.tile_count, t.reps, t.stride, tile_sub, last, gate);
        break;
    case TilePath::Matrix:
        hipLaunchKernelGGL(k_tile_scatter_matrix, dim3(tile_count_grid(grid)), dim3(kTBlock * kCountFold), lds, st, in.vals,
                           in.slots, in.nslots, per_read, ntiles, t.tile_base, t.matrix, t.stride, t.bucket, cov, ucov, tile_sub);
        break;
    case TilePath::TwoLevel:
        hipLaunchKernelGGL(k_part_super, dim3(grid), dim3(kTBlock), 0, st, in.vals, in.slots, in.nslots, per_read, ntiles,
                           t.tile_base, t.sup_cursor, t.mid, cov, ucov, tile_sub);
        hipLaunchKernelGGL(k_part_tile, dim3(part_items_upper(ntiles, n_upper)), dim3(kTBlock), 0, st, t.mid, t.part_items,
                           t.counters, t.tile_base, t.tile_cursor, ntiles, t.bucket);
        break;
    case TilePath::DirectAtomics:
        break;
    }
}

void launch_tile_fit(hipStream_t st, uint32_t ntiles, const TileTables& t, uint32_t* cov, uint32_t* ucov, uint32_t tile_sub,
                     const TileSample& sm) {
    const uint32_t peak = CNT_PEAK + (sm.flag - CNT_FALLBACK);
    hipLaunchKernelGGL(k_tile_fit, dim3(std::min(ntiles, 256u)), dim3(1024), 0, st, t.tile_count, t.tile_base, t.tile_cursor,
                       ntiles, t.stride, t.tile_items, t.split_tiles, t.counters, cov, ucov, tile_sub, sm.flag, peak);
}

uint32_t tile_items_upper(uint32_t ntiles, uint32_t n_upper) { return ntiles + n_upper / std::min(kTileSub, kTileSubB) + 1; }

void launch_tile_hist(hipStream_t st, uint32_t ntiles, uint32_t n_upper, const TileTables& t, uint32_t* cov, uint32_t* ucov,
                      const uint32_t* bin_off, uint32_t n_refs, uint32_t* stats, const BitsLayout& bits, uint32_t store_from,
                      bool wide, bool stretched) {
    const uint32_t grid = tile_items_upper(ntiles, n_upper);
    const uint32_t* const rb = stretched ? t.tile_count : nullptr;
    const uint32_t* const rf = stretched ? t.tile_cursor : nullptr;
    if (ucov && wide)
        hipLaunchKernelGGL((k_tile_hist<true, false>), dim3(grid), dim3(hist_block<true, false>()), 0, st, t.bucket, t.tile_items, t.counters, cov, ucov, bin_off,
                           n_refs, t.tile_ref0, stats, bits, store_from, rb, rf, t.stride);
    else if (ucov)
        hipLaunchKernelGGL((k_tile_hist<true, true>), dim3(grid), dim3(hist_block<true, true>()), 0, st, t.bucket, t.tile_items, t.counters, cov, ucov, bin_off,
                           n_refs, t.tile_ref0, stats, bits, store_from, rb, rf, t.stride);
    else
        hipLaunchKernelGGL((k_tile_hist<false, false>), dim3(grid), dim3(hist_block<false, false>()), 0, st, t.bucket, t.tile_items, t.counters, cov, cov, bin_off,
                           n_refs, t.tile_ref0, stats, bits, store_from, rb, rf, t.stride);
}

}
}

#ifndef TPROF_SHIFT
#define TPROF_SHIFT 13
#endif
#if defined(EXP) && (EXP == 8 || EXP == 9) && SLIMM_TILE_SHIFT == TPROF_SHIFT
extern "C" int slimm_debug_prof_tiles(unsigned long long* out, int n, int reset) {
    hipError_t e = hipMemcpyFromSymbol(out, HIP_SYMBOL(slimm::SLIMM_TILE_NS::g_prof_t), sizeof(unsigned long long) * n);
    if (reset) {
        static unsigned long long z[8 * 4096];
        (void)hipMemcpyToSymbol(HIP_SYMBOL(slimm::SLIMM_TILE_NS::g_prof_t), z, sizeof(z));
    }
    return e == hipSuccess ? 0 : -1;
}
#endif
```

slimm_amd/csrc/tile_plan.h:

```cpp
#pragma once
#include <algorithm>
#include <cstddef>
#include <cstdint>

#include "force.h"

namespace slimm {

constexpr uint32_t kTileShiftSmall = 13, kTileShiftLarge = 14;
constexpr uint32_t kTileSub = 49152;
constexpr uint32_t kTileSubB = 16384;
constexpr uint32_t kTileSubWide = 262144;
constexpr size_t kTileLdsMax = 144 * 1024;
inline bool tile_tables_fit_lds(uint32_t ntiles) { return static_cast<size_t>(ntiles) * 4 <= kTileLdsMax; }
#ifndef SLIMM_TILE_REPS
#define SLIMM_TILE_REPS 8
#endif
constexpr uint32_t kTileReps = SLIMM_TILE_REPS;
constexpr uint32_t kScanStagedTiles = 16384;
constexpr uint32_t kBigRoundTiles = 6144;
constexpr uint32_t kFusedScanTiles = 4064;

#if defined(__HIPCC__)
#define SLIMM_HD __host__ __device__
#else
#define SLIMM_HD
#endif
constexpr uint32_t kSampleMaxStride = 16;
constexpr uint32_t kSampleK = 8;
constexpr uint32_t kSamplePerStride = 1024;
constexpr uint64_t kSampleMinSkipped = 112000000ull;
SLIMM_HD inline uint64_t tile_isqrt_up(uint64_t x) {
    uint64_t r = static_cast<uint64_t>(__builtin_sqrt(static_cast<double>(x)));
    while (r * r > x) --r;
    while ((r + 1) * (r + 1) <= x) ++r;
    return r * r < x ? r + 1 : r;
}
SLIMM_HD inline uint32_t tile_isqrt_up32(uint32_t x) {
    uint32_t r = static_cast<uint32_t>(__builtin_sqrtf(static_cast<float>(x)));
    while (r * r > x) --r;
    while ((r + 1u) * (r + 1u) <= x) ++r;
    return r * r < x ? r + 1u : r;
}
SLIMM_HD inline uint32_t tile_cap(uint32_t c, uint32_t S, uint32_t k) {
    if (c >= (1u << 28)) return 0xffffffffu;
    const uint32_t r = tile_isqrt_up32(4u * c + k * k);
    const uint64_t cap = static_cast<uint64_t>(S) * c + (S * k * k + 1u) / 2u + (k * S * r + 1u) / 2u + S;
    return cap > 0xffffffffull ? 0xffffffffu : static_cast<uint32_t>(cap);
}
SLIMM_HD inline uint32_t tile_sample_first(uint32_t wave, uint32_t waves, uint32_t S) { return wave + waves * ((S - wave % S) % S); }
SLIMM_HD inline uint32_t tile_sample_step(uint32_t waves, uint32_t S) { return waves * S; }
inline uint32_t tile_sample_stride(uint64_t values, uint32_t ntiles) {
    const uint64_t per = values / (static_cast<uint64_t>(kTileReps) * std::max(1u, ntiles));
    uint32_t S = kSampleMaxStride;
    while (S > 1 && per < static_cast<uint64_t>(kSamplePerStride) * S) S >>= 1;
    return S;
}
inline uint64_t tile_cap_slack(uint64_t values, uint64_t stretches, uint32_t S, uint32_t k) {
    if (S <= 1) return 0;
    const uint64_t est = values + k * tile_isqrt_up(S * values);
    const uint64_t roots = tile_isqrt_up(stretches * (4 * est / S + 4 + static_cast<uint64_t>(k) * k * stretches)) + stretches;
    return (est - values) + (static_cast<uint64_t>(k) * S * roots + 1) / 2 + (static_cast<uint64_t>(S) * k * k / 2 + S + 2) * stretches;
}

struct TileLayout {
    uint32_t tile_shift = kTileShiftSmall;
    uint64_t Bp = 0;
    uint32_t ntiles = 0;
    uint32_t Tpad = 0, ntiles2 = 0;
    uint32_t tile_bins() const { return 1u << tile_shift; }
};
inline TileLayout tile_layout(uint64_t bins, uint32_t Tsel, long forced_shift = 0) {
    TileLayout l;
    const uint64_t small = (bins + (1ull << kTileShiftSmall) - 1) >> kTileShiftSmall;
    const uint64_t small2 = small + ((static_cast<uint64_t>(Tsel) + (1ull << kTileShiftSmall) - 1) >> kTileShiftSmall);
    l.tile_shift = small2 > kFusedScanTiles ? kTileShiftLarge : kTileShiftSmall;
    if (forced_shift == kTileShiftSmall || forced_shift == kTileShiftLarge) l.tile_shift = static_cast<uint32_t>(forced_shift);
    const uint32_t tb = l.tile_bins();
    l.Bp = (bins + tb - 1) & ~static_cast<uint64_t>(tb - 1);
    l.ntiles = static_cast<uint32_t>(l.Bp >> l.tile_shift);
    l.Tpad = (Tsel + tb - 1) & ~(tb - 1);
    l.ntiles2 = l.ntiles + (l.Tpad >> l.tile_shift);
    return l;
}

struct TileForces {
    bool direct_atomics = false;
    int two_level = -1;
    long fused_scan = 1;
    long matrix = 1;
    long scatter_big = 1;
    int wide_tiles = -1;
    long tile_shift = 0;
    long sample_stride = 0;
    long sample_k = -1;
    long bucket_room = 0;
    static TileForces from_env() {
        TileForces f;
        long v = 0;
        f.direct_atomics = forced("direct_atomics");
        if (forced("two_level", &v)) f.two_level = v == 1;
        (void)forced("fused_scan", &f.fused_scan);
        (void)forced("matrix", &f.matrix);
        (void)forced("scatter_big", &f.scatter_big);
        if (forced("wide_tiles", &v)) f.wide_tiles = v == 1;
        (void)forced("tile_shift", &f.tile_shift);
        (void)forced("sample_stride", &f.sample_stride);
        (void)forced("sample_k", &f.sample_k);
        (void)forced("bucket_room", &f.bucket_room);
        return f;
    }
};

struct TilePlan {
    bool use_tiles = false;
    bool two_level = false;
    uint32_t reps = 1, stride = 0;
    bool fused = false;
    bool matrix_allowed = false;
    bool matrix_always = false, scatter_big = true;
    int wide_tiles = -1;
    uint32_t sample_stride = 0, sample_k = kSampleK;
    uint64_t bucket_room = 0;
};
inline TilePlan tile_plan(uint32_t ntiles2, const TileForces& f, bool setup_ok) {
    TilePlan p;
    p.use_tiles = !f.direct_atomics && setup_ok;
    p.two_level = f.two_level >= 0 ? f.two_level == 1 : ntiles2 > kScanStagedTiles;
    if (!p.use_tiles) return p;
    p.reps = (p.two_level || ntiles2 > kScanStagedTiles) ? 1u : kTileReps;
    p.stride = ntiles2 + 1;
    p.fused = !p.two_level && p.reps == kTileReps && ntiles2 <= kFusedScanTiles && f.fused_scan != 0;
    p.matrix_allowed = !p.fused && f.matrix != 0 && (ntiles2 > kBigRoundTiles || f.matrix == 2);
    p.matrix_always = f.matrix == 2;
    p.scatter_big = f.scatter_big != 0;
    p.wide_tiles = f.wide_tiles;
    p.sample_stride = static_cast<uint32_t>(std::min<long>(std::max<long>(f.sample_stride, 0), kSampleMaxStride));
    if (f.sample_k >= 0) p.sample_k = static_cast<uint32_t>(std::min<long>(f.sample_k, 64));
    p.bucket_room = f.bucket_room > 0 ? static_cast<uint64_t>(f.bucket_room) : 0;
    return p;
}

enum class TilePhase { A, B };
enum class TilePath {
    DirectAtomics,
    Fused,
    OrderedRounds,
    DirectRounds,
    Matrix,
    TwoLevel
};
enum TileTable : uint32_t { kTabCount = 1, kTabBase = 2, kTabCursor = 4, kTabItems = 8, kTabBucket = 16, kTabMatrix = 32, kTabSuper = 64 };
struct TileRun {
    TilePhase phase = TilePhase::A;
    TilePath path = TilePath::DirectAtomics;
    uint32_t ntiles = 0;
    uint32_t scan_reps = 1;
    bool scan_two_level = false;
    uint32_t tile_sub = kTileSub;
    bool wide_hist = false;
    uint32_t tables = 0, zeroed = 0;
    uint32_t sample = 1;
    uint32_t sample_k = kSampleK;
};
inline bool tile_path_samples(const TilePlan& p, TilePath path, uint32_t ntiles) {
    return (path == TilePath::OrderedRounds || path == TilePath::DirectRounds) && p.reps == kTileReps && ntiles <= kScanStagedTiles;
}
inline TileRun tile_run(const TileLayout& l, const TilePlan& p, TilePhase phase, uint64_t values, uint64_t records) {
    TileRun r;
    const bool B = phase == TilePhase::B;
    r.phase = phase;
    r.ntiles = B ? l.ntiles2 : l.ntiles;
    if (!p.use_tiles) return r;
    const bool matrix = B && p.matrix_allowed && (p.matrix_always || values / std::max(1u, l.ntiles2) < 4096u);
    const bool ordered = p.scatter_big && p.reps > 1 && r.ntiles <= kBigRoundTiles;
    r.path = p.fused ? TilePath::Fused : matrix ? TilePath::Matrix : p.two_level ? TilePath::TwoLevel
             : ordered ? TilePath::OrderedRounds : TilePath::DirectRounds;
    r.scan_reps = matrix ? 1u : p.reps;
    r.scan_two_level = !matrix && p.two_level;
    const bool wide = p.wide_tiles >= 0 ? p.wide_tiles != 0 : (l.ntiles && records / l.ntiles > 32768u);
    r.tile_sub = wide ? kTileSubWide : (B ? kTileSubB : kTileSub);
    r.wide_hist = wide && !B;
    r.tables = kTabCount | kTabItems | kTabBucket | (p.fused ? 0u : kTabBase) | (matrix ? kTabMatrix : kTabCursor) |
               (r.path == TilePath::TwoLevel ? kTabSuper : 0u);
    r.zeroed = kTabCount | (p.fused ? kTabCursor : 0u);
    r.sample_k = p.sample_k;
    if (tile_path_samples(p, r.path, r.ntiles))
        r.sample = p.sample_stride ? p.sample_stride : tile_sample_stride(values, r.ntiles);
    if (!p.sample_stride && r.sample > 1 && values - values / r.sample < kSampleMinSkipped) r.sample = 1;
    return r;
}

inline uint64_t tile_bucket_entries(const TileLayout& l, const TilePlan& p, uint64_t n) {
    if (p.bucket_room) return p.bucket_room;
    uint64_t slack = 0;
    for (TilePhase ph : {TilePhase::A, TilePhase::B}) {
        const TileRun r = tile_run(l, p, ph, n, n);
        slack = std::max(slack, tile_cap_slack(n, static_cast<uint64_t>(kTileReps) * r.ntiles, r.sample, r.sample_k));
    }
    return n + 1 + slack;
}

}
```

Measured before the change: 115,400.

## Make tile histogram persistent with ticketed work stealing and prefetch

The histogram kernel becomes persistent. Its grid is capped at CUs times resident workgroups, and blocks pull items through an atomic ticket counter. Each block prefetches the next item's metadata into double-buffered LDS and clears its LDS accumulators in place instead of re-zeroing them per launch-block. The fit kernel now spreads its overflow check across all blocks and finishes with a last-block-done ticket, and a smaller scatter variant is used when the tile count is low. This trades launch and zeroing overhead for atomic ticket traffic and extra synchronisation per item.

New measurement: 114,700. No clear change (-0.6%).

```diff
diff --git a/slimm_amd/csrc/kernels.h b/slimm_amd/csrc/kernels.h
--- a/slimm_amd/csrc/kernels.h
+++ b/slimm_amd/csrc/kernels.h
@@ -30,6 +30,8 @@
     CNT_SPLIT = 9,
     CNT_FALLBACK = 11,
     CNT_PEAK = 13,
+    CNT_TICKET = 15,
+    CNT_FIT_DONE = 16,
     CNT_WORDS = 32
 };
 enum { ERR_REF_RANGE = 1, ERR_RUN_LENGTH = 2, ERR_PAIR_OVERFLOW = 4, ERR_KEY_COLLISION = 8 };
diff --git a/slimm_amd/csrc/tile_api.inc b/slimm_amd/csrc/tile_api.inc
--- a/slimm_amd/csrc/tile_api.inc
+++ b/slimm_amd/csrc/tile_api.inc
@@ -1,7 +1,7 @@
 int tile_hist_setup(uint32_t ntiles);
 uint32_t tile_count_grid(uint32_t grid);
 uint32_t part_items_upper(uint32_t ntiles, uint32_t n_upper);
-uint32_t tile_items_upper(uint32_t ntiles, uint32_t n_upper);
+uint32_t tile_items_upper(uint32_t ntiles, uint32_t n_upper, uint32_t tile_sub);
 void launch_tile_count(hipStream_t st, uint32_t grid, uint32_t ntiles, const SlotValues& in, const TileTables& t, bool totals,
                        bool matrix, const TileSample& sm = TileSample());
 void launch_matrix_prefix(hipStream_t st, uint32_t grid, uint32_t ntiles, const TileTables& t);
@@ -14,7 +14,7 @@
                      const TileSample& sm);
 void launch_tile_hist(hipStream_t st, uint32_t ntiles, uint32_t n_upper, const TileTables& t, uint32_t* cov, uint32_t* ucov,
                       const uint32_t* bin_off, uint32_t n_refs, uint32_t* stats, const BitsLayout& bits, uint32_t store_from,
-                      bool wide, bool stretched = false);
+                      bool wide, bool stretched, uint32_t tile_sub, uint32_t grid_forced = 0);
 void launch_pack(hipStream_t st, uint32_t* dst, const PackArgs& pack, const TileTables* t = nullptr, const uint32_t* a = nullptr,
                  const uint32_t* b = nullptr, const uint32_t* bin_off = nullptr, uint32_t n_refs = 0, uint32_t* stats = nullptr,
                  const BitsLayout& bits = BitsLayout());
diff --git a/slimm_amd/csrc/tile_bucketing.hip b/slimm_amd/csrc/tile_bucketing.hip
--- a/slimm_amd/csrc/tile_bucketing.hip
+++ b/slimm_amd/csrc/tile_bucketing.hip
@@ -29,7 +29,8 @@
     if (e != hipSuccess || !plan.use_tiles) return e;
     entries = static_cast<uint32_t>(std::min<uint64_t>(tile_bucket_entries(layout, plan, n), 0xffffffffull));
     if ((e = bucket.ensure(entries)) != hipSuccess || (e = mid.ensure(n + 1)) != hipSuccess) return e;
-    if ((e = tile_items.ensure(TILES(layout.tile_shift, tile_items_upper(layout.ntiles2, n)) + 1)) != hipSuccess) return e;
+    const uint32_t sub = std::min(tile_run(layout, plan, TilePhase::A, n, n).tile_sub, tile_run(layout, plan, TilePhase::B, n, n).tile_sub);
+    if ((e = tile_items.ensure(TILES(layout.tile_shift, tile_items_upper(layout.ntiles2, n, sub)) + 1)) != hipSuccess) return e;
     if ((e = part_items.ensure(TILES(layout.tile_shift, part_items_upper(layout.ntiles2, n)) + 1)) != hipSuccess) return e;
     return sup_cursor.ensure(kMaxSuper);
 }
@@ -76,8 +77,9 @@
     const TileRun& r = job.run;
     KernelTimer tm(c, r.phase == TilePhase::B ? K_TILE_HIST2 : K_TILE_HIST);
     const TileTables t = c->tiles.tables(c->counters.p);
-    TILES(t.tile_shift, launch_tile_hist(c->stream, r.ntiles, job.n_upper, t, job.a, job.b, c->d_bin_off.p, c->R, job.stats, job.bits,
-                                         job.store_from, r.wide_hist, r.sample > 1));
+    const uint32_t n_upper = job.values.slots ? job.n_upper : std::min(job.n_upper, job.values.nslots);
+    TILES(t.tile_shift, launch_tile_hist(c->stream, r.ntiles, n_upper, t, job.a, job.b, c->d_bin_off.p, c->R, job.stats, job.bits,
+                                         job.store_from, r.wide_hist, r.sample > 1, r.tile_sub, c->tiles.plan.hist_grid));
 }
 
 }
diff --git a/slimm_amd/csrc/tile_hist.hip b/slimm_amd/csrc/tile_hist.hip
--- a/slimm_amd/csrc/tile_hist.hip
+++ b/slimm_amd/csrc/tile_hist.hip
@@ -3,6 +3,7 @@
 #include <stdint.h>
 
 #include <algorithm>
+#include <atomic>
 
 #include "kernels.h"
 
@@ -466,6 +467,7 @@
     if (tid == 1023) {
         tile_base[ntiles] = carry.x;
         counters[CNT_ITEMS] = sampled ? 0u : carry.y;
+        counters[CNT_TICKET] = 0u;
         if (sampled) counters[flag] = s_caps > entries ? 1u : 0u;
     }
     __shared__ uint32_t s_n2;
@@ -822,6 +824,7 @@
 constexpr int kBigE = 6;
 static_assert(big_lds_bytes(kBigE) <= 160u * 1024u - 256u, "the two tables and the stage share a CU's LDS");
 static_assert(kBigE * kBigBlock == kBigRoundTiles, "kernels.h tells the context which layouts take these rounds");
+constexpr int kBigESmall = 5;
 static_assert(kTileShift + 1 + 14 <= 32, "a stage entry holds the tile and the bucket entry");
 
 __global__ __launch_bounds__(kTBlock * kCountFold) void k_tile_scatter_matrix(
@@ -963,6 +966,7 @@
         __syncthreads();
         if (tid == 0) {
             counters[CNT_ITEMS] = n_items;
+            counters[CNT_TICKET] = 0u;
             counters[CNT_ITEMS2] = 0;
             counters[CNT_SPLIT] = s_nsplit;
         }
@@ -1063,44 +1067,45 @@
 __global__ __launch_bounds__(1024) void k_tile_fit(uint32_t* rep_base, const uint32_t* __restrict__ tile_base,
                                                    const uint32_t* __restrict__ cursor,
                                                    uint32_t ntiles, uint32_t rep_stride, uint4* __restrict__ items,
-                                                   uint32_t* __restrict__ split_tiles, uint32_t* __restrict__ counters,
+                                                   uint32_t* __restrict__ split_tiles, uint32_t* counters,
                                                    uint32_t* __restrict__ cov, uint32_t* __restrict__ ucov, uint32_t tile_sub,
                                                    uint32_t flag, uint32_t peak) {
     __shared__ uint32_t s_cnt[kScanStaged];
     __shared__ uint2 s_wave[16];
-    __shared__ uint32_t s_over, s_peak, s_nsplit;
+    __shared__ uint32_t s_over, s_peak, s_nsplit, s_last;
     const uint32_t tid = threadIdx.x;
     const uint32_t raised = counters[flag];
-    if (blockIdx.x == 0) {
-        if (tid == 0) s_over = 0u, s_peak = 0u, s_nsplit = 0u;
-        __syncthreads();
+    const uint32_t share = (ntiles + gridDim.x - 1u) / gridDim.x;
+    const uint32_t t_lo = min(ntiles, blockIdx.x * share), t_hi = min(ntiles, t_lo + share);
+    if (tid == 0) s_over = 0u, s_peak = 0u, s_nsplit = 0u;
+    __syncthreads();
+    {
         uint32_t over = 0u, pk = 0u;
-        for (uint32_t i = tid; i < ntiles; i += 1024u) {
-            uint32_t b[kTileReps + 1], f[kTileReps], c = 0;
-#pragma unroll
-            for (uint32_t rep = 0; rep < kTileReps; ++rep) {
-                b[rep] = rep_base[static_cast<size_t>(rep) * rep_stride + i];
-                f[rep] = cursor[static_cast<size_t>(rep) * rep_stride + i];
-            }
-            b[kTileReps] = tile_base[i + 1];
-#pragma unroll
-            for (uint32_t rep = 0; rep < kTileReps; ++rep) {
-                const uint32_t cap = b[rep + 1] - b[rep];
-                if (f[rep] > cap) over = 1u;
-                if (f[rep]) pk = max(pk, static_cast<uint32_t>(min(4.0e9f, 1024.0f * static_cast<float>(f[rep]) / static_cast<float>(max(cap, 1u)))));
-                c += f[rep];
-            }
-            s_cnt[i] = c;
+        for (uint32_t j = tid; j < (t_hi - t_lo) * kTileReps; j += 1024u) {
+            const uint32_t i = t_lo + j / kTileReps, rep = j % kTileReps;
+            const uint32_t b0 = rep_base[static_cast<size_t>(rep) * rep_stride + i];
+            const uint32_t b1 = rep + 1u < kTileReps ? rep_base[static_cast<size_t>(rep + 1u) * rep_stride + i] : tile_base[i + 1];
+            const uint32_t f = cursor[static_cast<size_t>(rep) * rep_stride + i];
+            const uint32_t cap = b1 - b0;
+            if (f > cap) over = 1u;
+            if (f) pk = max(pk, static_cast<uint32_t>(min(4.0e9f, 1024.0f * static_cast<float>(f) / static_cast<float>(max(cap, 1u)))));
         }
         if (over) atomicOr(&s_over, 1u);
         if (pk) atomicMax(&s_peak, pk);
         __syncthreads();
-        if (tid == 0) counters[peak] = s_peak;
-        if (raised | s_over) {
-            if (tid == 0) counters[flag] = 1u;
-            for (uint32_t i = tid; i < kTileReps * rep_stride; i += 1024u) rep_base[i] = 0u;
-            return;
-        }
+        if (tid == 0) {
+            if (s_over) atomicOr(&counters[flag], 1u);
+            if (s_peak) atomicMax(&counters[peak], s_peak);
+        }
+    }
+    if (blockIdx.x == 0 && !raised) {
+        for (uint32_t i = tid; i < ntiles; i += 1024u) {
+            uint32_t c = 0;
+#pragma unroll
+            for (uint32_t rep = 0; rep < kTileReps; ++rep) c += cursor[static_cast<size_t>(rep) * rep_stride + i];
+            s_cnt[i] = c;
+        }
+        __syncthreads();
         const uint32_t per = (ntiles + 1023u) / 1024u;
         const uint32_t lo = min(tid * per, ntiles), hi = min(lo + per, ntiles);
         uint32_t mine = 0;
@@ -1134,17 +1139,17 @@
         __syncthreads();
         if (tid == 0) {
             counters[CNT_ITEMS] = total;
+            counters[CNT_TICKET] = 0u;
             counters[CNT_SPLIT] = s_nsplit;
         }
     }
     __shared__ uint32_t s_zero[64], s_nzero;
-    const uint32_t share = (ntiles + gridDim.x - 1u) / gridDim.x;
-    for (uint32_t t0 = blockIdx.x * share; t0 < min(ntiles, (blockIdx.x + 1u) * share); t0 += 64u) {
+    for (uint32_t t0 = t_lo; t0 < t_hi; t0 += 64u) {
         __syncthreads();
         if (tid == 0) s_nzero = 0u;
         __syncthreads();
         const uint32_t mine = t0 + tid;
-        if (tid < 64u && mine < min(ntiles, (blockIdx.x + 1u) * share)) {
+        if (tid < 64u && mine < t_hi) {
             uint32_t c = 0;
 #pragma unroll
             for (uint32_t rep = 0; rep < kTileReps; ++rep) c += cursor[static_cast<size_t>(rep) * rep_stride + mine];
@@ -1162,6 +1167,15 @@
             }
         }
     }
+    __threadfence();
+    __syncthreads();
+    if (tid == 0) s_last = atomicAdd(&counters[CNT_FIT_DONE], 1u) == gridDim.x - 1u ? 1u : 0u;
+    __syncthreads();
+    if (!s_last) return;
+    if (atomicOr(&counters[flag], 0u)) {
+        for (uint32_t i = tid; i < kTileReps * rep_stride; i += 1024u) rep_base[i] = 0u;
+    }
+    if (tid == 0) counters[CNT_FIT_DONE] = 0u;
 }
 
 constexpr uint32_t kPackWords = kTileBins / 2;
@@ -1188,8 +1202,9 @@
 }
 
 template <bool kPacked, uint32_t kWaves>
-__device__ __forceinline__ void tile_nonzero_bits(const uint32_t* s_a, uint32_t tile, const BitsLayout& bl, uint32_t array) {
-    const uint32_t lane = threadIdx.x & 63u, wave = threadIdx.x >> 6;
+__device__ __forceinline__ void tile_nonzero_bits(const uint32_t* s_a, uint32_t tile, const BitsLayout& bl, uint32_t array,
+                                                  uint32_t tid = threadIdx.x) {
+    const uint32_t lane = tid & 63u, wave = tid >> 6;
     uint64_t* dst = bl.base + (static_cast<uint64_t>(tile / bl.tps) * 2 + array) * bl.slice_w64 +
                     static_cast<uint64_t>(tile % bl.tps) * (kTileBins / 64);
     constexpr uint32_t kPart = kTileBins / kWaves;
@@ -1207,8 +1222,9 @@
 __device__ __forceinline__ void tile_ref_stats(const uint32_t* s_a, const uint32_t* s_b, uint32_t tile,
                                                const uint32_t* s_off, uint32_t r0,
                                                const uint32_t* __restrict__ bin_off, uint32_t n_refs,
-                                               uint32_t* __restrict__ stats, bool want_sum, bool want_nz) {
-    const uint32_t lane = threadIdx.x & 63u, wave = threadIdx.x >> 6;
+                                               uint32_t* __restrict__ stats, bool want_sum, bool want_nz,
+                                               uint32_t tid = threadIdx.x) {
+    const uint32_t lane = tid & 63u, wave = tid >> 6;
     const uint32_t tile0 = tile * kTileBins;
     const uint32_t t0 = tile0 + wave * (kTileBins / kWaves), t1 = t0 + kTileBins / kWaves;
     static_assert(kTileBins / kWaves <= 32768, "the two non-zero counts of a wave's part share one reduction");
@@ -1276,13 +1292,16 @@
 template <bool kTwo, bool kPacked>
 constexpr uint32_t hist_block() { return hist_lds_bytes<kTwo, kPacked>() > 64u * 1024u ? 1024u : 512u; }
 template <bool kTwo, bool kPacked>
-constexpr uint32_t hist_waves_per_simd() {
-    constexpr uint32_t wgs = std::min<uint32_t>(4u, (160u * 1024u) / (hist_lds_bytes<kTwo, kPacked>() + 1024u));
-    return wgs * (hist_block<kTwo, kPacked>() / 64u) / 4u;
-}
+constexpr uint32_t hist_wgs_per_cu() { return std::min<uint32_t>(4u, (160u * 1024u) / (hist_lds_bytes<kTwo, kPacked>() + 1024u)); }
+template <bool kTwo, bool kPacked>
+constexpr uint32_t hist_waves_per_simd() { return hist_wgs_per_cu<kTwo, kPacked>() * (hist_block<kTwo, kPacked>() / 64u) / 4u; }
+struct HistTabs {
+    uint32_t sb[kTileReps], sf[kTileReps], r0;
+};
+constexpr uint32_t kNextWords = 4u + 2u * kTileReps + 1u;
 template <bool kTwo, bool kPacked>
 __global__ __launch_bounds__((hist_block<kTwo, kPacked>()), (hist_waves_per_simd<kTwo, kPacked>())) void k_tile_hist(const uint16_t* __restrict__ bucket, const uint4* __restrict__ items,
-                                                   const uint32_t* __restrict__ counters, uint32_t* __restrict__ cov,
+                                                   uint32_t* counters, uint32_t* __restrict__ cov,
                                                    uint32_t* __restrict__ ucov, const uint32_t* __restrict__ bin_off,
                                                    uint32_t n_refs, const uint32_t* __restrict__ tile_ref0,
                                                    uint32_t* __restrict__ stats, const BitsLayout bits, uint32_t store_from,
@@ -1294,9 +1313,67 @@
     __shared__ uint32_t s_cov[kWords];
     __shared__ uint32_t s_ucov[kTwo ? kWords : 4];
     __shared__ uint32_t s_off[kStatRefs + 1];
+    __shared__ uint32_t s_ticket[2];
+    __shared__ uint32_t s_next[2][kNextWords];
+    uint32_t* const ticket = counters + CNT_TICKET;
+    const uint32_t n_items = __builtin_amdgcn_readfirstlane(counters[CNT_ITEMS]);
+    uint32_t tk_ahead = 0u;
+    if (threadIdx.x == 0) {
+        s_ticket[0] = atomicAdd(ticket, 1u);
+        tk_ahead = atomicAdd(ticket, 1u);
+    }
+    {
+        uint4* zc = reinterpret_cast<uint4*>(s_cov);
+        uint4* zu = reinterpret_cast<uint4*>(s_ucov);
+        const uint4 z = make_uint4(0, 0, 0, 0);
+        for (uint32_t i = threadIdx.x; i < kWords / 4; i += kHB) {
+            zc[i] = z;
+            if (kTwo) zu[i] = z;
+        }
+    }
+    __syncthreads();
+    auto item_word = [&](uint32_t i) -> uint32_t {
+        const uint32_t j = threadIdx.x;
+        if (j >= kNextWords) return 0u;
+        if (i >= n_items) return j == 3u ? 1u : 0u;
+        return reinterpret_cast<const uint32_t*>(items)[static_cast<size_t>(i) * 4 + (j < 4u ? j : 0u)];
+    };
+    auto next_word = [&](uint32_t iw, bool live) -> uint32_t {
+        const uint32_t j = threadIdx.x;
+        if (j < 4u || j >= kNextWords) return iw;
+        const uint32_t k = j - 4u;
+        if (k == 2u * kTileReps) return live && stats ? tile_ref0[iw] : n_refs;
+        if (!live || !rep_base) return 0u;
+        return (k < kTileReps ? rep_base : rep_fill)[static_cast<size_t>(k % kTileReps) * rep_stride + iw];
+    };
+    auto take = [&](uint32_t slot, uint4& item, HistTabs& t) {
+        const uint32_t* w = s_next[slot];
+        item.x = __builtin_amdgcn_readfirstlane(w[0]);
+        item.y = __builtin_amdgcn_readfirstlane(w[1]);
+        item.z = __builtin_amdgcn_readfirstlane(w[2]);
+        item.w = __builtin_amdgcn_readfirstlane(w[3]);
+#pragma unroll
+        for (uint32_t rep = 0; rep < kTileReps; ++rep) {
+            t.sb[rep] = rep_base ? __builtin_amdgcn_readfirstlane(w[4u + rep]) : 0u;
+            t.sf[rep] = rep_base ? __builtin_amdgcn_readfirstlane(w[4u + kTileReps + rep]) : 0u;
+        }
+        t.r0 = __builtin_amdgcn_readfirstlane(w[4u + 2u * kTileReps]);
+    };
+    uint32_t cur = __builtin_amdgcn_readfirstlane(s_ticket[0]);
+    {
+        const uint32_t pw = next_word(item_word(cur), cur < n_items);
+        if (threadIdx.x < kNextWords) s_next[0][threadIdx.x] = pw;
+        __syncthreads();
+    }
+    uint4 it;
+    HistTabs tb;
+    for (uint32_t par = 0; cur < n_items; par ^= 1u) {
     HPROF_T(h0);
-    if (blockIdx.x >= counters[CNT_ITEMS]) return;
-    const uint4 it = items[blockIdx.x];
+    uint32_t tid = threadIdx.x;
+    SLIMM_PIN_VGPR(tid);
+    take(par, it, tb);
+    const uint32_t tk = tk_ahead;
+    if (tid == 0) tk_ahead = atomicAdd(ticket, 1u);
     const uint32_t tile = it.x, lo = it.y, hi = it.z;
     const bool whole = it.w == 1;
     if (whole && lo == hi) {
@@ -1304,37 +1381,27 @@
             uint4* oc = reinterpret_cast<uint4*>(cov + static_cast<size_t>(tile) * kTileBins);
             uint4* ou = reinterpret_cast<uint4*>(ucov + static_cast<size_t>(tile) * kTileBins);
             const uint4 z = make_uint4(0, 0, 0, 0);
-            for (uint32_t i = threadIdx.x; i < kTileBins / 4; i += kHB) {
+            for (uint32_t i = tid; i < kTileBins / 4; i += kHB) {
                 oc[i] = z;
                 if (kTwo) ou[i] = z;
             }
         }
-        if (bits.base && threadIdx.x < kTileBins / 64) {
+        if (bits.base && tid < kTileBins / 64) {
             for (uint32_t array = 0; array < (kTwo ? 2u : 1u); ++array)
                 bits.base[(static_cast<uint64_t>(tile / bits.tps) * 2 + array) * bits.slice_w64 +
-                          static_cast<uint64_t>(tile % bits.tps) * (kTileBins / 64) + threadIdx.x] = 0ull;
-        }
-        return;
-    }
-    uint32_t sb[kTileReps], sf[kTileReps];
-#pragma unroll
-    for (uint32_t rep = 0; rep < kTileReps; ++rep) {
-        sb[rep] = rep_base ? rep_base[static_cast<size_t>(rep) * rep_stride + tile] : 0u;
-        sf[rep] = rep_base ? rep_fill[static_cast<size_t>(rep) * rep_stride + tile] : 0u;
-    }
-    const uint32_t r0 = stats ? tile_ref0[tile] : n_refs;
-    const bool stage_off = threadIdx.x <= kStatRefs && r0 < n_refs && r0 + threadIdx.x <= n_refs;
-    const uint32_t off_reg = stage_off ? bin_off[r0 + threadIdx.x] : 0u;
-    {
-        uint4* zc = reinterpret_cast<uint4*>(s_cov);
-        uint4* zu = reinterpret_cast<uint4*>(s_ucov);
-        const uint4 z = make_uint4(0, 0, 0, 0);
-        for (uint32_t i = threadIdx.x; i < kWords / 4; i += kHB) {
-            zc[i] = z;
-            if (kTwo) zu[i] = z;
-        }
-    }
-    __syncthreads();
+                          static_cast<uint64_t>(tile % bits.tps) * (kTileBins / 64) + tid] = 0ull;
+        }
+        if (tid == 0) s_ticket[par ^ 1u] = tk;
+        __syncthreads();
+        cur = __builtin_amdgcn_readfirstlane(s_ticket[par ^ 1u]);
+        const uint32_t pw = next_word(item_word(cur), cur < n_items);
+        if (tid < kNextWords) s_next[par ^ 1u][tid] = pw;
+        __syncthreads();
+        continue;
+    }
+    const uint32_t r0 = tb.r0;
+    const bool stage_off = tid <= kStatRefs && r0 < n_refs && r0 + tid <= n_refs;
+    const uint32_t off_reg = stage_off ? bin_off[r0 + tid] : 0u;
     HPROF_T(h2);
     HPROF_ADD(1, h0, h2);
     {
@@ -1346,19 +1413,19 @@
             const uint32_t a0 = min(hi, (lo + 7u) & ~7u);
             const uint32_t n8 = (hi - a0) >> 3;
             const uint32_t a1 = a0 + (n8 << 3);
-            if (lo + threadIdx.x < a0) one(bucket[lo + threadIdx.x]);
-            if (a1 + threadIdx.x < hi) one(bucket[a1 + threadIdx.x]);
+            if (lo + tid < a0) one(bucket[lo + tid]);
+            if (a1 + tid < hi) one(bucket[a1 + tid]);
             const uint4* __restrict__ b8 = reinterpret_cast<const uint4*>(bucket + a0);
             for (uint32_t i0 = 0; i0 < n8; i0 += 2 * kHB) {
                 uint4 q[2];
 #pragma unroll
                 for (int u = 0; u < 2; ++u) {
-                    const uint32_t i = i0 + u * kHB + threadIdx.x;
+                    const uint32_t i = i0 + u * kHB + tid;
                     q[u] = i < n8 ? b8[i] : make_uint4(0xffffffffu, 0xffffffffu, 0xffffffffu, 0xffffffffu);
                 }
 #pragma unroll
                 for (int u = 0; u < 2; ++u) {
-                    if (i0 + u * kHB + threadIdx.x >= n8) continue;
+                    if (i0 + u * kHB + tid >= n8) continue;
                     const uint32_t w[4] = {q[u].x, q[u].y, q[u].z, q[u].w};
 #pragma unroll
                     for (int k = 0; k < 4; ++k) {
@@ -1368,8 +1435,8 @@
                 }
             }
         } else {
-            const uint32_t(&b)[kTileReps] = sb;
-            const uint32_t(&f)[kTileReps] = sf;
+            const uint32_t(&b)[kTileReps] = tb.sb;
+            const uint32_t(&f)[kTileReps] = tb.sf;
             static_assert(kHB >= 16u * kTileReps, "sixteen threads per stretch take its ragged ends");
             uint32_t first[kTileReps], pre[kTileReps + 1];
             uint32_t p = 0, ev = 0xffffffffu;
@@ -1381,8 +1448,8 @@
                 const uint32_t a0 = min(shi, (slo + 7u) & ~7u), n8 = (shi - a0) >> 3, a1 = a0 + (n8 << 3);
                 first[rep] = a0;
                 pre[rep + 1] = pre[rep] + n8;
-                if ((threadIdx.x >> 4) == rep) {
-                    const uint32_t sub = threadIdx.x & 15u;
+                if ((tid >> 4) == rep) {
+                    const uint32_t sub = tid & 15u;
                     const uint32_t at = sub < 8u ? slo + sub : a1 + (sub - 8u), end = sub < 8u ? a0 : shi;
                     if (at < end) ev = bucket[at];
                 }
@@ -1393,7 +1460,7 @@
                 uint4 q[2];
 #pragma unroll
                 for (int u = 0; u < 2; ++u) {
-                    const uint32_t g = i0 + u * kHB + threadIdx.x;
+                    const uint32_t g = i0 + u * kHB + tid;
                     uint32_t at = first[0], g0 = 0u;
 #pragma unroll
                     for (uint32_t rep = 1; rep < kTileReps; ++rep)
@@ -1404,7 +1471,7 @@
                 if (i0 == 0u && ev != 0xffffffffu) one(ev);
 #pragma unroll
                 for (int u = 0; u < 2; ++u) {
-                    if (i0 + u * kHB + threadIdx.x >= groups) continue;
+                    if (i0 + u * kHB + tid >= groups) continue;
                     const uint32_t w[4] = {q[u].x, q[u].y, q[u].z, q[u].w};
 #pragma unroll
                     for (int k = 0; k < 4; ++k) {
@@ -1418,65 +1485,102 @@
     }
     HPROF_T(h3);
     HPROF_ADD(2, h2, h3);
-    if (stage_off) s_off[threadIdx.x] = off_reg;
+    if (stage_off) s_off[tid] = off_reg;
+    if (tid == 0) s_ticket[par ^ 1u] = tk;
     __syncthreads();
     HPROF_T(h4);
     HPROF_ADD(3, h3, h4);
+    const uint32_t nxt = __builtin_amdgcn_readfirstlane(s_ticket[par ^ 1u]);
+    const uint32_t iw = item_word(nxt);
     uint32_t* gc = cov + static_cast<size_t>(tile) * kTileBins;
     uint32_t* gu = ucov + static_cast<size_t>(tile) * kTileBins;
+    if (stats) tile_ref_stats<kTwo, kPacked, kWaves>(s_cov, s_ucov, tile, s_off, r0, bin_off, n_refs, stats, true, whole, tid);
+    HPROF_T(h5);
+    HPROF_ADD(4, h4, h5);
+    const uint32_t pw = next_word(iw, nxt < n_items);
+    const uint32_t lane = tid & 63u, wave = tid >> 6;
+    constexpr uint32_t kPart = kTileBins / kWaves;
     if (whole) {
         uint4* oc = reinterpret_cast<uint4*>(gc);
         uint4* ou = reinterpret_cast<uint4*>(gu);
-        const uint4* sc = reinterpret_cast<const uint4*>(s_cov);
-        const uint4* su = reinterpret_cast<const uint4*>(s_ucov);
-        if (stats) tile_ref_stats<kTwo, kPacked, kWaves>(s_cov, s_ucov, tile, s_off, r0, bin_off, n_refs, stats, true, true);
-        HPROF_T(h5);
-        HPROF_ADD(4, h4, h5);
-        if (tile >= store_from && !kPacked) {
-            for (uint32_t i = threadIdx.x; i < kTileBins / 4; i += kHB) {
-                oc[i] = sc[i];
-                if (kTwo) ou[i] = su[i];
-            }
-        } else if (tile >= store_from) {
-            for (uint32_t i = threadIdx.x; i < kPackWords / 4; i += kHB) {
+        uint4* sc = reinterpret_cast<uint4*>(s_cov);
+        uint4* su = reinterpret_cast<uint4*>(s_ucov);
+        const uint4 z = make_uint4(0, 0, 0, 0);
+        if (bits.base) {
+            tile_nonzero_bits<kPacked, kWaves>(s_cov, tile, bits, 0, tid);
+            if (kTwo) tile_nonzero_bits<kPacked, kWaves>(s_ucov, tile, bits, 1, tid);
+        }
+        if (kPacked) __syncthreads();
+        if (tile < store_from) {
+            for (uint32_t i = kPacked ? tid : wave * (kPart / 4) + lane; i < (kPacked ? kWords / 4 : (wave + 1u) * (kPart / 4));
+                 i += kPacked ? kHB : 64u) {
+                sc[i] = z;
+                if (kTwo) su[i] = z;
+            }
+        } else if (!kPacked) {
+            for (uint32_t i = wave * (kPart / 4) + lane; i < (wave + 1u) * (kPart / 4); i += 64u) {
                 const uint4 w = sc[i];
+                sc[i] = z;
+                oc[i] = w;
+                if (kTwo) {
+                    const uint4 x = su[i];
+                    su[i] = z;
+                    ou[i] = x;
+                }
+            }
+        } else {
+            for (uint32_t i = tid; i < kPackWords / 4; i += kHB) {
+                const uint4 w = sc[i];
+                sc[i] = z;
                 oc[i] = make_uint4(w.x & 0xffffu, w.y & 0xffffu, w.z & 0xffffu, w.w & 0xffffu);
                 oc[i + kPackWords / 4] = make_uint4(w.x >> 16, w.y >> 16, w.z >> 16, w.w >> 16);
                 if (kTwo) {
                     const uint4 x = su[i];
+                    su[i] = z;
                     ou[i] = make_uint4(x.x & 0xffffu, x.y & 0xffffu, x.z & 0xffffu, x.w & 0xffffu);
                     ou[i + kPackWords / 4] = make_uint4(x.x >> 16, x.y >> 16, x.z >> 16, x.w >> 16);
                 }
             }
         }
-        if (bits.base) {
-            tile_nonzero_bits<kPacked, kWaves>(s_cov, tile, bits, 0);
-            if (kTwo) tile_nonzero_bits<kPacked, kWaves>(s_ucov, tile, bits, 1);
-        }
-        HPROF_T(h6);
-        HPROF_ADD(5, h5, h6);
-        HPROF_ADD(7, h0, h6);
-        return;
-    }
-    for (uint32_t i = threadIdx.x; !kPacked && i < kTileBins; i += kHB) {
-        const uint32_t a = s_cov[i];
-        if (a) atomicAdd(&gc[i], a);
-        if (kTwo) {
-            const uint32_t b2 = s_ucov[i];
-            if (b2) atomicAdd(&gu[i], b2);
-        }
-    }
-    for (uint32_t i = threadIdx.x; kPacked && i < kPackWords; i += kHB) {
-        const uint32_t a = s_cov[i];
-        if (a & 0xffffu) atomicAdd(&gc[i], a & 0xffffu);
-        if (a >> 16) atomicAdd(&gc[i + kPackWords], a >> 16);
-        if (kTwo) {
-            const uint32_t b2 = s_ucov[i];
-            if (b2 & 0xffffu) atomicAdd(&gu[i], b2 & 0xffffu);
-            if (b2 >> 16) atomicAdd(&gu[i + kPackWords], b2 >> 16);
-        }
-    }
-    if (stats) tile_ref_stats<kTwo, kPacked, kWaves>(s_cov, s_ucov, tile, s_off, r0, bin_off, n_refs, stats, true, false);
+    } else {
+        if (kPacked) __syncthreads();
+        for (uint32_t i = wave * kPart + lane; !kPacked && i < (wave + 1u) * kPart; i += 64u) {
+            const uint32_t a = s_cov[i];
+            if (a) {
+                s_cov[i] = 0u;
+                atomicAdd(&gc[i], a);
+            }
+            if (kTwo) {
+                const uint32_t b2 = s_ucov[i];
+                if (b2) {
+                    s_ucov[i] = 0u;
+                    atomicAdd(&gu[i], b2);
+                }
+            }
+        }
+        for (uint32_t i = tid; kPacked && i < kPackWords; i += kHB) {
+            const uint32_t a = s_cov[i];
+            if (a) s_cov[i] = 0u;
+            if (a & 0xffffu) atomicAdd(&gc[i], a & 0xffffu);
+            if (a >> 16) atomicAdd(&gc[i + kPackWords], a >> 16);
+            if (kTwo) {
+                const uint32_t b2 = s_ucov[i];
+                if (b2) s_ucov[i] = 0u;
+                if (b2 & 0xffffu) atomicAdd(&gu[i], b2 & 0xffffu);
+                if (b2 >> 16) atomicAdd(&gu[i + kPackWords], b2 >> 16);
+            }
+        }
+    }
+    HPROF_T(h6);
+    HPROF_ADD(5, h5, h6);
+    if (tid < kNextWords) s_next[par ^ 1u][tid] = pw;
+    __syncthreads();
+    HPROF_T(h7);
+    HPROF_ADD(6, h6, h7);
+    HPROF_ADD(7, h0, h7);
+    HPROF_ADD(0, 0ull, 1ull);
+    cur = nxt;
+    }
 }
 
 template <bool kTwo>
@@ -1552,6 +1656,9 @@
     if (hipFuncSetAttribute(reinterpret_cast<const void*>(k_tile_scatter_big<kBigE>), hipFuncAttributeMaxDynamicSharedMemorySize,
                             static_cast<int>(big_lds_bytes(kBigE))) != hipSuccess)
         return -1;
+    if (hipFuncSetAttribute(reinterpret_cast<const void*>(k_tile_scatter_big<kBigESmall>), hipFuncAttributeMaxDynamicSharedMemorySize,
+                            static_cast<int>(big_lds_bytes(kBigESmall))) != hipSuccess)
+        return -1;
     return 0;
 }
 
@@ -1595,9 +1702,14 @@
                            t.split_tiles, tot.part, tot.nparts, tot.tail, tile_sub);
         break;
     case TilePath::OrderedRounds:
-        hipLaunchKernelGGL(k_tile_scatter_big<kBigE>, dim3(tile_count_grid(grid)), dim3(kBigBlock), big_lds_bytes(kBigE), st,
-                           in.vals, in.slots, in.nslots, per_read, ntiles, t.tile_base, t.tile_cursor, t.bucket, cov, ucov,
-                           t.tile_count, t.reps, t.stride, tile_sub, last, gate);
+        if (ntiles <= static_cast<uint32_t>(kBigESmall) * kBigBlock)
+            hipLaunchKernelGGL(k_tile_scatter_big<kBigESmall>, dim3(tile_count_grid(grid)), dim3(kBigBlock), big_lds_bytes(kBigESmall),
+                               st, in.vals, in.slots, in.nslots, per_read, ntiles, t.tile_base, t.tile_cursor, t.bucket, cov, ucov,
+                               t.tile_count, t.reps, t.stride, tile_sub, last, gate);
+        else
+            hipLaunchKernelGGL(k_tile_scatter_big<kBigE>, dim3(tile_count_grid(grid)), dim3(kBigBlock), big_lds_bytes(kBigE), st,
+                               in.vals, in.slots, in.nslots, per_read, ntiles, t.tile_base, t.tile_cursor, t.bucket, cov, ucov,
+                               t.tile_count, t.reps, t.stride, tile_sub, last, gate);
         break;
     case TilePath::DirectRounds:
         hipLaunchKernelGGL(k_tile_scatter, dim3(grid), dim3(kTBlock), lds, st, in.vals, in.slots, in.nslots, per_read, ntiles,
@@ -1625,12 +1737,25 @@
                        ntiles, t.stride, t.tile_items, t.split_tiles, t.counters, cov, ucov, tile_sub, sm.flag, peak);
 }
 
-uint32_t tile_items_upper(uint32_t ntiles, uint32_t n_upper) { return ntiles + n_upper / std::min(kTileSub, kTileSubB) + 1; }
+uint32_t tile_items_upper(uint32_t ntiles, uint32_t n_upper, uint32_t tile_sub) { return ntiles + n_upper / std::max(tile_sub, 1u) + 1; }
+
+static uint32_t hist_cus() {
+    static std::atomic<uint32_t> cus[64];
+    int dev = 0, v = 0;
+    if (hipGetDevice(&dev) != hipSuccess || dev < 0 || dev >= 64) dev = 0;
+    uint32_t n = cus[dev].load(std::memory_order_relaxed);
+    if (!n) {
+        if (hipDeviceGetAttribute(&v, hipDeviceAttributeMultiprocessorCount, dev) != hipSuccess || v <= 0) v = 256;
+        cus[dev].store(n = static_cast<uint32_t>(v), std::memory_order_relaxed);
+    }
+    return n;
+}
 
 void launch_tile_hist(hipStream_t st, uint32_t ntiles, uint32_t n_upper, const TileTables& t, uint32_t* cov, uint32_t* ucov,
                       const uint32_t* bin_off, uint32_t n_refs, uint32_t* stats, const BitsLayout& bits, uint32_t store_from,
-                      bool wide, bool stretched) {
-    const uint32_t grid = tile_items_upper(ntiles, n_upper);
+                      bool wide, bool stretched, uint32_t tile_sub, uint32_t grid_forced) {
+    const uint32_t per_cu = ucov && wide ? hist_wgs_per_cu<true, false>() : ucov ? hist_wgs_per_cu<true, true>() : hist_wgs_per_cu<false, false>();
+    const uint32_t grid = grid_forced ? grid_forced : std::min(hist_cus() * per_cu, tile_items_upper(ntiles, n_upper, tile_sub));
     const uint32_t* const rb = stretched ? t.tile_count : nullptr;
     const uint32_t* const rf = stretched ? t.tile_cursor : nullptr;
     if (ucov && wide)
diff --git a/slimm_amd/csrc/tile_plan.h b/slimm_amd/csrc/tile_plan.h
--- a/slimm_amd/csrc/tile_plan.h
+++ b/slimm_amd/csrc/tile_plan.h
@@ -95,6 +95,7 @@
     long sample_stride = 0;
     long sample_k = -1;
     long bucket_room = 0;
+    long hist_grid = 0;
     static TileForces from_env() {
         TileForces f;
         long v = 0;
@@ -108,6 +109,7 @@
         (void)forced("sample_stride", &f.sample_stride);
         (void)forced("sample_k", &f.sample_k);
         (void)forced("bucket_room", &f.bucket_room);
+        (void)forced("hist_grid", &f.hist_grid);
         return f;
     }
 };
@@ -122,6 +124,7 @@
     int wide_tiles = -1;
     uint32_t sample_stride = 0, sample_k = kSampleK;
     uint64_t bucket_room = 0;
+    uint32_t hist_grid = 0;
 };
 inline TilePlan tile_plan(uint32_t ntiles2, const TileForces& f, bool setup_ok) {
     TilePlan p;
@@ -138,6 +141,7 @@
     p.sample_stride = static_cast<uint32_t>(std::min<long>(std::max<long>(f.sample_stride, 0), kSampleMaxStride));
     if (f.sample_k >= 0) p.sample_k = static_cast<uint32_t>(std::min<long>(f.sample_k, 64));
     p.bucket_room = f.bucket_room > 0 ? static_cast<uint64_t>(f.bucket_room) : 0;
+    p.hist_grid = static_cast<uint32_t>(std::min<long>(std::max<long>(f.hist_grid, 0), 65535));
     return p;
 }
 
```
